# Edresson/VoiceSplit

Measured on AMD Instinct MI355X. Metric: utterances/sec (3 s clips, B=64/GPU) fwd+bwd, channels-last bf16 activations / tape, bf16 MFMA, fp32 accumulate / statistics / master weights, higher is better.
Workload: dtype bf16 (conv activations and tape stored as bf16; bf16 MFMA operands in the convs, the LSTM / head contractions and the BPTT, f16 operands in the forward recurrence; fp32 accumulate, BatchNorm statistics, gate arithmetic / cell state, loss head, master weights)

## Files before the change

### voicesplit_amd/csrc/audio.hip

```cpp
#include <math.h>

#include "../../include/voicesplit_hip.h"
#include "stft_common.h"

namespace {

__global__ __launch_bounds__(256)
void reim_to_features_kernel(const float* __restrict__ reim, float* __restrict__ spec, float* __restrict__ phase, VsStftShape s) {
  const long long n = (long long)s.B * s.T * s.F;
  for (long long i = (long long)blockIdx.x * 256 + threadIdx.x; i < n; i += (long long)gridDim.x * 256) {
    const long long m = i / s.F;
    const int f = (int)(i - m * s.F);
    const float re = reim[m * s.ldk + f], im = reim[m * s.ldk + s.F + f];
    const float mag = sqrtf(re * re + im * im);
    const float db = 20.0f * log10f(fmaxf(1e-5f, mag)) - s.ref_level_db;
    spec[i] = fminf(fmaxf(db / (-s.min_level_db), -1.0f), 0.0f) + 1.0f;
    if (phase) phase[i] = atan2f(im, re);
  }
}

}

extern "C" {

size_t vs_audio_workspace_bytes(const vs_loss_dims* d) { return vs_sisnr_workspace_bytes(d); }

int vs_wav_to_spec(const vs_loss_dims* d, const float* wav, float* spec, float* phase, void* ws, size_t ws_bytes, void* stream_) {
  hipStream_t stream = (hipStream_t)stream_;
  VsStftShape s;
  if (int rc = vs_stft_make_shape(d, &s)) return rc;
  s.periodic = 1;
  const VsStftLayout L = vs_stft_layout(s);
  VS_REQUIRE(wav && spec, "wav_to_spec: NULL argument");
  VS_REQUIRE(s.S > s.n_fft / 2, "wav_to_spec: clip shorter than the reflect padding");
  VS_REQUIRE(ws && (reinterpret_cast<uintptr_t>(ws) & 255) == 0 && ws_bytes >= L.total, "wav_to_spec: workspace too small or misaligned (%zu < %zu)", ws_bytes, L.total);
  const int M = s.B * s.T;
  float* frames = at<float>(ws, L.frames_e);
  float* basis = at<float>(ws, L.fbasis);
  float* reim = at<float>(ws, L.reim_e);
  const bool split = vs_stft_split(s);
  unsigned* amax = at<unsigned>(ws, L.amax);
  float* scales = at<float>(ws, L.scales);
  if (split) VS_CHECK_HIP(hipMemsetAsync(amax, 0, (size_t)VS_AMAX_SLOTS * 4, stream));
  vs_stft_frames_launch(wav, frames, s, split ? amax : nullptr, vs_grid_for((long long)M * s.win, split ? 2048 : 16384), stream);
  vs_stft_basis_launch(basis, s, scales + 6, stream);
  if (split) if (int rc = vs_scale_from_absmax_impl(amax, VS_AMAX_SLOTS, scales, stream)) return rc;
  if (int rc = vs_stft_contract(split, 0, frames, s.win, basis, s.win, reim, s.ldk, M, s.K, s.win, scales, scales + 6, stream)) return rc;
  hipLaunchKernelGGL(reim_to_features_kernel, dim3(vs_grid_for((long long)M * s.F, 16384)), dim3(256), 0, stream, reim, spec, phase, s);
  VS_LAUNCH_CHECK();
  return 0;
}

int vs_spec_to_wav(const vs_loss_dims* d, const float* spec, const float* mask, const float* phase, float* wav,
                   void* ws, size_t ws_bytes, void* stream_) {
  hipStream_t stream = (hipStream_t)stream_;
  VsStftShape s;
  if (int rc = vs_stft_make_shape(d, &s)) return rc;
  s.periodic = 1;
  s.true_phase = 1;
  const VsStftLayout L = vs_stft_layout(s);
  VS_REQUIRE(spec && phase && wav, "spec_to_wav: NULL argument");
  if (int rc = vs_stft_check_envelope(s)) return rc;
  VS_REQUIRE(ws && (reinterpret_cast<uintptr_t>(ws) & 255) == 0 && ws_bytes >= L.total, "spec_to_wav: workspace too small or misaligned (%zu < %zu)", ws_bytes, L.total);
  const int M = s.B * s.T;
  float* basis = at<float>(ws, L.basis);
  float* env = at<float>(ws, L.env);
  float* reim = at<float>(ws, L.reim_e);
  float* frames = at<float>(ws, L.frames_e);
  const bool split = vs_stft_split(s);
  unsigned* amax = at<unsigned>(ws, L.amax);
  float* scales = at<float>(ws, L.scales);
  vs_istft_basis_launch(basis, s, scales + 6, stream);
  vs_istft_envelope_launch(env, s, stream);
  if (split) VS_CHECK_HIP(hipMemsetAsync(amax, 0, (size_t)VS_AMAX_SLOTS * 4, stream));
  vs_spec_to_reim_launch(spec, mask, phase, reim, s, split ? amax : nullptr, vs_grid_for((long long)M * s.F, split ? 2048 : 16384), stream);
  if (split) if (int rc = vs_scale_from_absmax_impl(amax, VS_AMAX_SLOTS, scales, stream)) return rc;
  if (int rc = vs_stft_contract(split, 0, reim, s.ldk, basis, s.ldk, frames, s.win, M, s.win, s.K, scales, scales + 6, stream)) return rc;
  vs_overlap_add_launch(frames, env, wav, s, stream);
  VS_LAUNCH_CHECK();
  return 0;
}

}
```

### voicesplit_amd/csrc/conv_f16x3.hip

```cpp
#include "conv_f16x3_common.h"
#include "vs_internal.h"

namespace {

constexpr int kPadTaps = 2;

__global__ __launch_bounds__(256)
void absmax_kernel(const float* __restrict__ x, long long n, unsigned* __restrict__ out) {
  float m = 0.f;
  const long long n4 = n >> 2;
  const float4* x4 = reinterpret_cast<const float4*>(x);
  for (long long i = (long long)blockIdx.x * 256 + threadIdx.x; i < n4; i += (long long)gridDim.x * 256) {
    const float4 v = x4[i];
    m = fmaxf(m, fmaxf(fmaxf(fabsf(v.x), fabsf(v.y)), fmaxf(fabsf(v.z), fabsf(v.w))));
  }
  if (blockIdx.x == 0 && threadIdx.x < (n & 3)) m = fmaxf(m, fabsf(x[(n4 << 2) + threadIdx.x]));
#pragma unroll
  for (int o = 32; o > 0; o >>= 1) m = fmaxf(m, __shfl_down(m, o, 64));
  if ((threadIdx.x & 63) == 0) atomicMax(out, __float_as_uint(m));
}

__global__ void scale_from_absmax_kernel(const unsigned* __restrict__ amax, int n, float* __restrict__ scale) {
  unsigned mb = 0;
  for (int i = threadIdx.x; i < n; i += 64) mb = amax[i] > mb ? amax[i] : mb;
#pragma unroll
  for (int o = 32; o > 0; o >>= 1) { const unsigned other = __shfl_down(mb, o, 64); mb = other > mb ? other : mb; }
  if (threadIdx.x != 0) return;
  const float m = __uint_as_float(mb);
  int e = 0;
  float s = 1.f, inv = 1.f;
  if (m > 0.f && m < 3.0e38f) {
    (void)frexpf(m, &e);
    int k = 10 - e;
    k = k > 100 ? 100 : (k < -100 ? -100 : k);
    s = ldexpf(1.f, k);
    inv = ldexpf(1.f, -k);
  }
  scale[0] = s;
  scale[1] = inv;
}

__global__ void conv_pack_weights_f16_kernel(const float* __restrict__ w, _Float16* __restrict__ wp, int KT, int KF,
                                             int transpose_flip, const float* __restrict__ wscale) {
  const int NT = KT * KF;
  const int total = kNChunk * NT * 2 * 2 * 64 * 8;
  int idx = blockIdx.x * blockDim.x + threadIdx.x;
  if (idx >= total + kPadTaps * (kTapBytes / 2)) return;
  if (idx >= total) { wp[idx] = (_Float16)0.f; return; }
  const int j = idx & 7;
  const int lane = (idx >> 3) & 63;
  const int part = (idx >> 9) & 1;
  const int cb = (idx >> 10) & 1;
  const int tg = idx >> 11;
  const int chunk = tg / NT, tap = tg - chunk * NT;
  const int kt = tap / KF, kf = tap - kt * KF;
  const int co = cb * 32 + (lane & 31);
  const int ci = chunk * kChunk + 8 * (lane >> 5) + j;
  const float v = (transpose_flip ? w[((ci * kCi + co) * KT + (KT - 1 - kt)) * KF + (KF - 1 - kf)]
                                  : w[((co * kCi + ci) * KT + kt) * KF + kf]) * wscale[0];
  f16x2 hi, lo;
  split2(v, 0.f, hi, lo);
  wp[idx] = part ? lo[0] : hi[0];
}

template <int KT, int KF, int P, int ACT, bool STATS = false>
__global__ __launch_bounds__(256, 2)
void conv64_f16x3_kernel(const float* __restrict__ in, const _Float16* __restrict__ wp,
                         const float* __restrict__ scale, const float* __restrict__ shift,
                         const float* __restrict__ in_scale, const float* __restrict__ w_scale,
                         float* __restrict__ out, int T, int F, int dil, int n_rt, int n_ft, unsigned* amax_out,
                         int i_base, int i_end,
                         double* bn_stats = nullptr) {
  constexpr int R = 4 * P;
  constexpr int ROWS = R + KT - 1;
  constexpr int PX = kTileF + KF - 1 + ((kTileF + KF - 1) % 4 ? 4 - (kTileF + KF - 1) % 4 : 0);
  constexpr int NPIX = ROWS * PX;
  constexpr int NPP = (NPIX + 255) / 256;
  constexpr int NT = KT * KF;
  constexpr int GT = KF == 1 ? KT : KF;
  constexpr int NGRP = NT / GT;
  __shared__ __attribute__((aligned(16))) u32x4 sIn[(NPIX + (P + 1) * PX) * 4];
  constexpr int NWBUF = NGRP > 1 ? 2 : 1;
  __shared__ __attribute__((aligned(16))) u32x4 sW[NWBUF][GT * kTapVec];

  const int tid = threadIdx.x;
  const int lane = tid & 63;
  const int wave = __builtin_amdgcn_readfirstlane(tid >> 6);
  const int l31 = lane & 31;
  const int half = lane >> 5;

  int bid = blockIdx.x;
  const int ft = bid % n_ft; bid /= n_ft;
  const int rt = bid % n_rt; bid /= n_rt;
  const int cls = bid % dil;
  const int b = bid / dil;
  const int n_all = (T - cls + dil - 1) / dil;
  const int n_c = n_all < i_end ? n_all : i_end;
  const int i0 = i_base + rt * R;
  if (i0 >= n_c) return;
  const int f0 = ft * kTileF;
  const size_t plane = (size_t)T * F;
  const float* in_b = in + (size_t)b * kCi * plane;
  const unsigned plane_bytes = (unsigned)(plane * sizeof(float));
  const unsigned slab_bytes = plane_bytes * kChunk;
  const float s_in = in_scale[0];
  const float inv = in_scale[1] * w_scale[1];

  unsigned voff[NPP];
#pragma unroll
  for (int i = 0; i < NPP; ++i) {
    const int pix = tid + 256 * i;
    const int rr = pix / PX;
    const int x = pix - rr * PX;
    const int iin = i0 - KT / 2 + rr;
    const int f = f0 - KF / 2 + x;
    const bool ok = (pix < NPIX) && (iin >= 0) && (iin < n_all) && (f >= 0) && (f < F);
    voff[i] = ok ? (unsigned)(((cls + dil * iin) * F + f) * 4) : kOob;
  }
  float stage[NPP][kChunk];
  auto load_chunk = [&](int chunk) {
    const float* src = in_b + (size_t)chunk * kChunk * plane;
    __amdgpu_buffer_rsrc_t rsrc = __builtin_amdgcn_make_buffer_rsrc(const_cast<float*>(src), 0, slab_bytes, 0x00020000);
#pragma unroll
    for (int i = 0; i < NPP; ++i)
#pragma unroll
      for (int c = 0; c < kChunk; ++c)
        stage[i][c] = __builtin_bit_cast(float, __builtin_amdgcn_raw_buffer_load_b32(rsrc, voff[i], c * plane_bytes, 0));
  };
  auto store_chunk = [&]() {
#pragma unroll
    for (int i = 0; i < NPP; ++i) {
      const int pix = tid + 256 * i;
      if (pix < NPIX) {
        const int sw = ((pix % PX) >> 2) & 3;
#pragma unroll
        for (int h = 0; h < 2; ++h) {
          f16x2 hi[4], lo[4];
#pragma unroll
          for (int q = 0; q < 4; ++q) split2(stage[i][8 * h + 2 * q] * s_in, stage[i][8 * h + 2 * q + 1] * s_in, hi[q], lo[q]);
          u32x4 vh, vl;
#pragma unroll
          for (int q = 0; q < 4; ++q) {
            vh[q] = __builtin_bit_cast(unsigned, hi[q]);
            vl[q] = __builtin_bit_cast(unsigned, lo[q]);
          }
          sIn[pix * 4 + ((0 + h) ^ sw)] = vh;
          sIn[pix * 4 + ((2 + h) ^ sw)] = vl;
        }
      }
    }
  };

  __amdgpu_buffer_rsrc_t wrsrc = __builtin_amdgcn_make_buffer_rsrc(
      const_cast<_Float16*>(wp), 0, (unsigned)((kNChunk * NT + kPadTaps) * kTapBytes), 0x00020000);
  u32x4 wreg[GT];
  auto load_w = [&](int gg) {
#pragma unroll
    for (int i = 0; i < GT; ++i)
      wreg[i] = __builtin_amdgcn_raw_buffer_load_b128(wrsrc, (unsigned)((tid + 256 * i) * 16), gg * (GT * kTapBytes), 0);
  };
  auto store_w = [&](int buf) {
#pragma unroll
    for (int i = 0; i < GT; ++i) sW[buf][tid + 256 * i] = wreg[i];
  };

  f32x16 acc[2][P];
#pragma unroll
  for (int cb = 0; cb < 2; ++cb)
#pragma unroll
    for (int p = 0; p < P; ++p)
#pragma unroll
      for (int r = 0; r < 16; ++r) acc[cb][p][r] = 0.f;

  const bool wave_active = (i0 + wave * P) < n_c;
  auto load_a = [&](int buf, int g, u32x4 (&a)[2][2]) {
#pragma unroll
    for (int cb = 0; cb < 2; ++cb)
#pragma unroll
      for (int part = 0; part < 2; ++part) a[cb][part] = sW[buf][g * kTapVec + (cb * 2 + part) * 64 + lane];
  };
  const u32x4* bbase[KF][2];
#pragma unroll
  for (int kf = 0; kf < KF; ++kf) {
    const int x = l31 + kf;
    const int sw = (x >> 2) & 3;
    bbase[kf][0] = sIn + ((wave * P) * PX + x) * 4 + ((0 + half) ^ sw);
    bbase[kf][1] = sIn + ((wave * P) * PX + x) * 4 + ((2 + half) ^ sw);
  }
  auto load_b = [&](int kt, int kf, u32x4 (&bf)[P][2]) {
#pragma unroll
    for (int p = 0; p < P; ++p) {
      bf[p][0] = bbase[kf][0][(p + kt) * PX * 4];
      bf[p][1] = bbase[kf][1][(p + kt) * PX * 4];
    }
  };

  load_w(0);
  load_chunk(0);
  int gg = 0;
#pragma unroll 1
  for (int chunk = 0; chunk < kNChunk; ++chunk) {
    __syncthreads();
    store_chunk();
#pragma unroll
    for (int grp = 0; grp < NGRP; ++grp, ++gg) {
      const int buf = NWBUF > 1 ? (gg & 1) : 0;
      store_w(buf);
      __syncthreads();
      if (gg + 1 < kNChunk * NGRP) load_w(gg + 1);
      if (grp == 0 && chunk + 1 < kNChunk) load_chunk(chunk + 1);
      if (wave_active) {
        u32x4 a_cur[2][2], a_nxt[2][2], b_cur[P][2], b_nxt[P][2];
        const int kt0 = KF == 1 ? 0 : grp;
        load_a(buf, 0, a_cur);
        load_b(kt0, 0, b_cur);
#pragma unroll
        for (int g = 0; g < GT; ++g) {
          const int gn = g + 1 < GT ? g + 1 : g;
          load_a(buf, gn, a_nxt);
          load_b(KF == 1 ? gn : kt0, KF == 1 ? 0 : gn, b_nxt);
          __builtin_amdgcn_sched_barrier(0);
#pragma unroll
          for (int term = 0; term < 3; ++term) {
#pragma unroll
            for (int p = 0; p < P; ++p) {
              const f16x8 bq = __builtin_bit_cast(f16x8, b_cur[p][term == 1 ? 1 : 0]);
#pragma unroll
              for (int cb = 0; cb < 2; ++cb) {
                const f16x8 aq = __builtin_bit_cast(f16x8, a_cur[cb][term == 0 ? 1 : 0]);
                acc[cb][p] = __builtin_amdgcn_mfma_f32_32x32x16_f16(aq, bq, acc[cb][p], 0, 0, 0);
              }
            }
          }
          __builtin_amdgcn_sched_barrier(0);
#pragma unroll
          for (int cb = 0; cb < 2; ++cb)
#pragma unroll
            for (int part = 0; part < 2; ++part) a_cur[cb][part] = a_nxt[cb][part];
#pragma unroll
          for (int p = 0; p < P; ++p) { b_cur[p][0] = b_nxt[p][0]; b_cur[p][1] = b_nxt[p][1]; }
        }
      }
    }
  }

  if (!STATS && !wave_active) return;
  const int f = f0 + l31;
  float* out_b = out + (size_t)b * kCo * plane;
  float m = 0.f;
  float stS[2][16], stQ[2][16];
#pragma unroll
  for (int cb = 0; cb < 2; ++cb) {
#pragma unroll
    for (int r = 0; r < 16; ++r) {
      const int co = cb * 32 + (r & 3) + 8 * (r >> 2) + 4 * half;
      const float sc = scale[co] * inv, sh = shift[co];
      stS[cb][r] = 0.f; stQ[cb][r] = 0.f;
#pragma unroll
      for (int p = 0; p < P; ++p) {
        const int i = i0 + wave * P + p;
        if (wave_active && i < n_c && f < F) {
          const int t = cls + dil * i;
          const float y = vs_act_fast<ACT>(fmaf(acc[cb][p][r], sc, sh));
          out_b[(size_t)co * plane + (size_t)t * F + f] = y;
          m = fmaxf(m, fabsf(y));
          if (STATS) { stS[cb][r] += y; stQ[cb][r] = fmaf(y, y, stQ[cb][r]); }
        }
      }
    }
  }
  vs_absmax_commit(m, amax_out);
  if (STATS) {
#pragma unroll
    for (int cb = 0; cb < 2; ++cb)
#pragma unroll
      for (int r = 0; r < 16; ++r) {
        float sv = stS[cb][r], qv = stQ[cb][r];
#pragma unroll
        for (int o = 16; o > 0; o >>= 1) { sv += __shfl_xor(sv, o, 64); qv += __shfl_xor(qv, o, 64); }
        stS[cb][r] = sv; stQ[cb][r] = qv;
      }
    __syncthreads();
    float* red = reinterpret_cast<float*>(sIn);
    if (l31 == 0) {
#pragma unroll
      for (int cb = 0; cb < 2; ++cb)
#pragma unroll
        for (int r = 0; r < 16; ++r) {
          const int co = cb * 32 + (r & 3) + 8 * (r >> 2) + 4 * half;
          red[(wave * 64 + co) * 2 + 0] = stS[cb][r];
          red[(wave * 64 + co) * 2 + 1] = stQ[cb][r];
        }
    }
    __syncthreads();
    if (tid < 128) {
      const double v = (double)red[tid] + (double)red[128 + tid] + (double)red[256 + tid] + (double)red[384 + tid];
      atomicAdd(bn_stats + (size_t)(blockIdx.x % VS_BN_STAT_SLOTS) * 128 + tid, v);
    }
  }
}

template <int KT, int KF, int P>
int launch_conv(const float* in, const _Float16* wp, const float* scale, const float* shift, const float* in_scale,
                const float* w_scale, float* out, int B, int T, int F, int dil, int act, unsigned* amax_out, hipStream_t stream,
                int i_base = 0, int i_end = 0x7fffffff, double* bn_stats = nullptr) {
  constexpr int R = 4 * P;
  const int rows_all = (T + dil - 1) / dil;
  const int rows_max = (rows_all < i_end ? rows_all : i_end) - i_base;
  const int n_rt = (rows_max + R - 1) / R;
  const int n_ft = (F + kTileF - 1) / kTileF;
  const long long nblk = (long long)B * dil * n_rt * n_ft;
  VS_REQUIRE(nblk > 0 && nblk < 2147483647LL, "conv64_f16x3: grid of %lld blocks out of range", nblk);
  dim3 grid((unsigned)nblk), block(256);
  auto launch = [&](auto A, auto S) {
    hipLaunchKernelGGL((conv64_f16x3_kernel<KT, KF, P, decltype(A)::value, decltype(S)::value>), grid, block, 0, stream, in, wp, scale, shift,
                       in_scale, w_scale, out, T, F, dil, n_rt, n_ft, amax_out, i_base, i_end, bn_stats);
  };
  if (bn_stats) {
    VS_REQUIRE(act == VS_ACT_NONE, "conv64_f16x3: fused BatchNorm statistics need act = NONE");
    launch(std::integral_constant<int, VS_ACT_NONE>(), std::true_type());
  } else if (int rc = conv_f16x3_dispatch_act(act, "conv64_f16x3", [&](auto A) { launch(A, std::false_type()); })) {
    return rc;
  }
  VS_LAUNCH_CHECK();
  return 0;
}

long long tile_rows(int T, int dil, int R) {
  long long tot = 0;
  for (int c = 0; c < dil && c < T; ++c) {
    int n = (T - c + dil - 1) / dil;
    tot += (long long)((n + R - 1) / R) * R;
  }
  return tot;
}

}

extern "C" size_t vs_conv64_packed_f16_floats(int KT, int KF) { return (size_t)(kNChunk * KT * KF + kPadTaps) * (kTapBytes / 4); }

int vs_scale_from_absmax_impl(const unsigned* amax, int n, float* scale2, hipStream_t stream) {
  hipLaunchKernelGGL(scale_from_absmax_kernel, dim3(1), dim3(64), 0, stream, amax, n, scale2);
  VS_LAUNCH_CHECK();
  return 0;
}

int vs_absmax_accum_impl(const float* x, long long n, unsigned* amax, hipStream_t stream) {
  VS_REQUIRE(n > 0, "absmax: n=%lld", n);
  VS_REQUIRE((reinterpret_cast<uintptr_t>(x) & 15) == 0, "absmax: tensor must be 16-byte aligned");
  const long long nb = ((n >> 2) + 255) / 256;
  hipLaunchKernelGGL(absmax_kernel, dim3((unsigned)(nb < 2048 ? (nb > 0 ? nb : 1) : 2048)), dim3(256), 0, stream, x, n, amax);
  VS_LAUNCH_CHECK();
  return 0;
}

int vs_pow2_scale_impl(const float* x, long long n, unsigned* amax_scratch, float* scale2, hipStream_t stream) {
  VS_REQUIRE(n > 0, "pow2_scale: n=%lld", n);
  VS_REQUIRE((reinterpret_cast<uintptr_t>(x) & 15) == 0, "pow2_scale: tensor must be 16-byte aligned");
  VS_CHECK_HIP(hipMemsetAsync(amax_scratch, 0, sizeof(unsigned), stream));
  const long long nb = ((n >> 2) + 255) / 256;
  hipLaunchKernelGGL(absmax_kernel, dim3((unsigned)(nb < 2048 ? (nb > 0 ? nb : 1) : 2048)), dim3(256), 0, stream, x, n, amax_scratch);
  return vs_scale_from_absmax_impl(amax_scratch, 1, scale2, stream);
}

int vs_conv64_pack_f16_impl(const float* w, _Float16* wp, int KT, int KF, int transpose_flip, unsigned* amax_scratch,
                            float* w_scale2, hipStream_t stream) {
  VS_REQUIRE((KT == 7 && KF == 1) || (KT == 5 && KF == 5), "conv64_f16x3: unsupported kernel %dx%d", KT, KF);
  if (int rc = vs_pow2_scale_impl(w, (long long)kCo * kCi * KT * KF, amax_scratch, w_scale2, stream)) return rc;
  const int total = (int)(vs_conv64_packed_f16_floats(KT, KF) * 2);
  hipLaunchKernelGGL(conv_pack_weights_f16_kernel, dim3((total + 255) / 256), dim3(256), 0, stream, w, wp, KT, KF, transpose_flip, w_scale2);
  VS_LAUNCH_CHECK();
  return 0;
}

static int g_conv_kernel = 0;
extern "C" int vs_set_conv_kernel(int mode) {
  if (mode < 0 || mode > 2) return -1;
  g_conv_kernel = mode;
  return 0;
}

int vs_conv64_f16x3_fwd_impl(const float* in, const _Float16* wp, const float* scale, const float* shift,
                             const float* in_scale2, const float* w_scale2, float* out,
                             int B, int T, int F, int KT, int KF, int dil, int act, unsigned* amax_out, hipStream_t stream,
                             double* bn_stats) {
  VS_REQUIRE(B > 0 && T > 0 && F > 0 && dil > 0, "conv64_f16x3: bad shape B=%d T=%d F=%d dil=%d", B, T, F, dil);
  VS_REQUIRE((long long)kChunk * T * F * 4 < (long long)kOob, "conv64_f16x3: T*F=%lld too large for 32-bit slab offsets", (long long)T * F);
  VS_REQUIRE((KT == 7 && KF == 1) || (KT == 5 && KF == 5), "conv64_f16x3: unsupported kernel %dx%d", KT, KF);
  const bool p2 = tile_rows(T, dil, 8) * 100 <= tile_rows(T, dil, 4) * 112;
  const int all = 0x7fffffff;
#define VS_ONE_TILE(KT_, KF_, P_, I0_, I1_) \
  launch_conv<KT_, KF_, P_>(in, wp, scale, shift, in_scale2, w_scale2, out, B, T, F, dil, act, amax_out, stream, I0_, I1_, bn_stats)
  if (KT == 7) return p2 ? VS_ONE_TILE(7, 1, 2, 0, all) : VS_ONE_TILE(7, 1, 1, 0, all);
  const int rows_all = (T + dil - 1) / dil, full8 = rows_all / 8 * 8, rem = rows_all - full8;
  const bool tail = full8 > 0 && rem > 0 && rem <= 4;
  const int body_end = tail ? full8 : all;
  int rc;
  if (g_conv_kernel != 1 && (long long)kCo * T * F * 4 < (long long)kOob) {
    rc = vs_conv64_f16x3_pk_impl(in, wp, scale, shift, in_scale2, w_scale2, out, B, T, F, dil, act, amax_out, stream,
                                 g_conv_kernel == 2 ? vs_opt(VS_OPT_ABLATION) : 0, body_end, bn_stats);
  } else {
    rc = tail || p2 ? VS_ONE_TILE(5, 5, 2, 0, body_end) : VS_ONE_TILE(5, 5, 1, 0, body_end);
  }
  if (rc || !tail) return rc;
  return VS_ONE_TILE(5, 5, 1, full8, all);
#undef VS_ONE_TILE
}
```

### voicesplit_amd/csrc/gemm_f16x3.hip

```cpp
#include <stdlib.h>

#include "vs_internal.h"

namespace {

typedef _Float16 h8 __attribute__((ext_vector_type(8)));
typedef _Float16 h2 __attribute__((ext_vector_type(2)));
typedef unsigned u2v __attribute__((ext_vector_type(2)));
typedef unsigned u4v __attribute__((ext_vector_type(4)));

constexpr int BM = 128, BN = 128;
constexpr int pitch_of(int BK) { return BK / 2 + 2; }
constexpr int regs_of(int BK) { return BM * BK / 256; }

struct Gemm16Args {
  const float* A; int lda;
  const float* W; int ldw;
  const float* W_hi; int n_split;
  float* C; int ldc;
  int M, N, K;
  const float* bias1;
  const float* bias2;
  const float* rowbias;
  int ldrb, group;
  const float* gate; int ldg;
  int a_relu, w_relu, act, accumulate;
  const float* a_scale;
  const float* w_scale;
  int tiles_m, tiles_n;
  int band;
};

template <bool BF = false>
__device__ __forceinline__ void split_pair(float x0, float x1, unsigned& hi, unsigned& lo) {
  if (BF) { hi = vs_pack_bf16(x0, x1); lo = 0u; return; }
  const h2 h = __builtin_bit_cast(h2, __builtin_amdgcn_cvt_pkrtz(x0, x1));
  const h2 l = __builtin_bit_cast(h2, __builtin_amdgcn_cvt_pkrtz(x0 - (float)h[0], x1 - (float)h[1]));
  hi = __builtin_bit_cast(unsigned, h);
  lo = __builtin_bit_cast(unsigned, l);
}

template <bool BF, class HV>
__device__ __forceinline__ f32x16 g_mma(HV a, HV b, f32x16 c, int, int, int) {
  if (BF) return __builtin_amdgcn_mfma_f32_32x32x16_bf16(__builtin_bit_cast(vs_bf16x8, a), __builtin_bit_cast(vs_bf16x8, b), c, 0, 0, 0);
  return __builtin_amdgcn_mfma_f32_32x32x16_f16(a, b, c, 0, 0, 0);
}

struct OperandView {
  __amdgpu_buffer_rsrc_t lo, hi;
  int row_lo, rows_lo;
  int row_hi, rows_hi;
  int use_lo, use_hi;
};

constexpr unsigned kOob = 0xFFFFFFF0u;

__device__ __forceinline__ bool gemm_tile_of(int tiles_m, int tiles_n, int band_rows, int& tm, int& tn) {
  const int per = (int)(gridDim.x >> 3);
  const int t = (int)(blockIdx.x & 7) * per + (int)(blockIdx.x >> 3);
  if (t >= tiles_m * tiles_n) return false;
  if (band_rows <= 0) { tm = t / tiles_n; tn = t - tm * tiles_n; return true; }
  const int band_tiles = band_rows * tiles_n;
  const int band = t / band_tiles;
  const int r = t - band * band_tiles;
  const int rows = min(band_rows, tiles_m - band * band_rows);
  tn = r / rows;
  tm = band * band_rows + (r - tn * rows);
  return true;
}

template <int LAYOUT, bool VEC, int BK>
__device__ __forceinline__ void tile_load(float (&r)[regs_of(BK)], const OperandView& o, int ld, int row0_kmajor, int k0, int K, int tid) {
  constexpr int RT = regs_of(BK);
  typedef float f4 __attribute__((ext_vector_type(4)));
  if (LAYOUT == 0) {
#pragma unroll
    for (int i = 0; i < RT / 4; ++i) {
      const int v = tid + 256 * i;
      const int lr = v / (BK / 4), c4 = k0 + (v % (BK / 4)) * 4;
      f4 t = {0.f, 0.f, 0.f, 0.f};
      auto fetch = [&](const __amdgpu_buffer_rsrc_t rs, int row, int nrows) {
        const bool okr = row >= 0 && row < nrows;
        const unsigned base = ((unsigned)row * (unsigned)ld + (unsigned)c4) * 4u;
        if (VEC) {
          return __builtin_bit_cast(f4, __builtin_amdgcn_raw_buffer_load_b128(rs, (okr && c4 < K) ? base : kOob, 0, 0));
        } else {
          f4 q;
#pragma unroll
          for (int e = 0; e < 4; ++e)
            q[e] = __builtin_bit_cast(float, __builtin_amdgcn_raw_buffer_load_b32(rs, (okr && c4 + e < K) ? base + 4u * e : kOob, 0, 0));
          return q;
        }
      };
      if (o.use_lo) t = fetch(o.lo, o.row_lo + lr, o.rows_lo);
      if (o.use_hi) t += fetch(o.hi, o.row_hi + lr, o.rows_hi);
      r[4 * i + 0] = t[0]; r[4 * i + 1] = t[1]; r[4 * i + 2] = t[2]; r[4 * i + 3] = t[3];
    }
  } else {
    const unsigned voff = ((unsigned)(2 * (tid >> 7)) * (unsigned)ld + (unsigned)(tid & 127)) * 4u;
    const unsigned so0 = ((unsigned)k0 * (unsigned)ld + (unsigned)row0_kmajor) * 4u;
#pragma unroll
    for (int i = 0; i < RT / 2; ++i) {
      const unsigned so = so0 + (unsigned)(4 * i) * (unsigned)ld * 4u;
      r[2 * i + 0] = __builtin_bit_cast(float, __builtin_amdgcn_raw_buffer_load_b32(o.lo, voff, so, 0));
      r[2 * i + 1] = __builtin_bit_cast(float, __builtin_amdgcn_raw_buffer_load_b32(o.lo, voff, so + (unsigned)ld * 4u, 0));
    }
  }
}

template <int LAYOUT, int BK, bool BF = false>
__device__ __forceinline__ void tile_store(const float (&r)[regs_of(BK)], unsigned* __restrict__ sh, unsigned* __restrict__ sl,
                                           float s, bool relu, int tid) {
  constexpr int RT = regs_of(BK), PW = pitch_of(BK);
  const float floor_ = relu ? 0.f : -__builtin_inff();
  if (LAYOUT == 0) {
#pragma unroll
    for (int i = 0; i < RT / 4; ++i) {
      const int v = tid + 256 * i;
      float x[4];
#pragma unroll
      for (int j = 0; j < 4; ++j) x[j] = fmaxf(r[4 * i + j], floor_) * s;
      unsigned h0, l0, h1, l1;
      split_pair<BF>(x[0], x[1], h0, l0);
      split_pair<BF>(x[2], x[3], h1, l1);
      u2v hi, lo;
      hi[0] = h0; hi[1] = h1;
      lo[0] = l0; lo[1] = l1;
      *reinterpret_cast<u2v*>(&sh[(v / (BK / 4)) * PW + (v % (BK / 4)) * 2]) = hi;
      *reinterpret_cast<u2v*>(&sl[(v / (BK / 4)) * PW + (v % (BK / 4)) * 2]) = lo;
    }
  } else {
#pragma unroll
    for (int i = 0; i < RT / 2; ++i) {
      const int idx = tid + 256 * i;
      const float x0 = fmaxf(r[2 * i], floor_) * s;
      const float x1 = fmaxf(r[2 * i + 1], floor_) * s;
      unsigned hi, lo;
      split_pair<BF>(x0, x1, hi, lo);
      sh[(idx & 127) * PW + (idx >> 7)] = hi;
      sl[(idx & 127) * PW + (idx >> 7)] = lo;
    }
  }
}

template <int LA, int LB, bool VEC, int BK, int OCC, bool BF = false>
__global__ __launch_bounds__(256, OCC)
void gemm_f16x3_kernel(Gemm16Args g) {
  constexpr int RT = regs_of(BK), PW = pitch_of(BK);
  __shared__ __attribute__((aligned(16))) unsigned sAh[BM * PW], sAl[BM * PW], sWh[BN * PW], sWl[BN * PW];

  const int tid = threadIdx.x;
  const int lane = tid & 63;
  const int wave = tid >> 6;
  const int wm = wave >> 1, wn = wave & 1;
  const int l31 = lane & 31, half = lane >> 5;
  int tile_m, tile_n;
  if (!gemm_tile_of(g.tiles_m, g.tiles_n, g.band, tile_m, tile_n)) return;
  const int m0 = tile_m * BM, n0 = tile_n * BN;
  const float sa = g.a_scale[0], sw = g.w_scale[0];
  const float inv = g.a_scale[1] * g.w_scale[1];

  f32x16 acc[2][2];
#pragma unroll
  for (int a = 0; a < 2; ++a)
#pragma unroll
    for (int b = 0; b < 2; ++b)
#pragma unroll
      for (int r = 0; r < 16; ++r) acc[a][b][r] = 0.f;

  float ra[RT], rw[RT];
  auto desc = [](const float* p, size_t floats) {
    return __builtin_amdgcn_make_buffer_rsrc(const_cast<float*>(p), 0, (int)(floats * 4), 0x00020000);
  };
  OperandView va, vw;
  va.lo = va.hi = desc(g.A, LA ? (size_t)(g.K - 1) * g.lda + g.M : (size_t)(g.M - 1) * g.lda + g.K);
  va.row_lo = m0; va.rows_lo = g.M; va.row_hi = 0; va.rows_hi = 0; va.use_lo = 1; va.use_hi = 0;
  const int nlo = g.n_split < g.N ? g.n_split : g.N;
  vw.lo = desc(g.W, LB ? (size_t)(g.K - 1) * g.ldw + g.N : (size_t)(nlo - 1) * g.ldw + g.K);
  vw.hi = (!LB && g.N > nlo) ? desc(g.W_hi, (size_t)(g.N - nlo - 1) * g.ldw + g.K) : vw.lo;
  vw.row_lo = n0; vw.rows_lo = nlo; vw.row_hi = n0 - nlo; vw.rows_hi = g.N - nlo;
  vw.use_lo = LB || n0 < nlo; vw.use_hi = !LB && n0 + BN > nlo && g.N > nlo;

  const int fa = (wm * 64 + l31) * PW + 4 * half;
  const int fw = (wn * 64 + l31) * PW + 4 * half;

  tile_load<LA, VEC, BK>(ra, va, g.lda, m0, 0, g.K, tid);
  tile_load<LB, VEC, BK>(rw, vw, g.ldw, n0, 0, g.K, tid);
  for (int k0 = 0; k0 < g.K; k0 += BK) {
    __syncthreads();
    tile_store<LA, BK, BF>(ra, sAh, sAl, sa, g.a_relu != 0, tid);
    tile_store<LB, BK, BF>(rw, sWh, sWl, sw, g.w_relu != 0, tid);
    __syncthreads();
    if (k0 + BK < g.K) {
      tile_load<LA, VEC, BK>(ra, va, g.lda, m0, k0 + BK, g.K, tid);
      tile_load<LB, VEC, BK>(rw, vw, g.ldw, n0, k0 + BK, g.K, tid);
    }
#pragma unroll
    for (int ks = 0; ks < BK / 16; ++ks) {
      h8 ah[2], al[2], bh[2], bl[2];
#pragma unroll
      for (int x = 0; x < 2; ++x) {
        const int oa = fa + x * 32 * PW + 8 * ks, ow = fw + x * 32 * PW + 8 * ks;
        u4v t;
        u2v p0 = *reinterpret_cast<const u2v*>(&sAh[oa]), p1 = *reinterpret_cast<const u2v*>(&sAh[oa + 2]);
        t[0] = p0[0]; t[1] = p0[1]; t[2] = p1[0]; t[3] = p1[1];
        ah[x] = __builtin_bit_cast(h8, t);
        p0 = *reinterpret_cast<const u2v*>(&sAl[oa]); p1 = *reinterpret_cast<const u2v*>(&sAl[oa + 2]);
        t[0] = p0[0]; t[1] = p0[1]; t[2] = p1[0]; t[3] = p1[1];
        al[x] = __builtin_bit_cast(h8, t);
        p0 = *reinterpret_cast<const u2v*>(&sWh[ow]); p1 = *reinterpret_cast<const u2v*>(&sWh[ow + 2]);
        t[0] = p0[0]; t[1] = p0[1]; t[2] = p1[0]; t[3] = p1[1];
        bh[x] = __builtin_bit_cast(h8, t);
        p0 = *reinterpret_cast<const u2v*>(&sWl[ow]); p1 = *reinterpret_cast<const u2v*>(&sWl[ow + 2]);
        t[0] = p0[0]; t[1] = p0[1]; t[2] = p1[0]; t[3] = p1[1];
        bl[x] = __builtin_bit_cast(h8, t);
      }
#pragma unroll
      for (int term = BF ? 2 : 0; term < 3; ++term)
#pragma unroll
        for (int mb = 0; mb < 2; ++mb)
#pragma unroll
          for (int nb = 0; nb < 2; ++nb)
            acc[mb][nb] = g_mma<BF>(term == 0 ? al[mb] : ah[mb], term == 1 ? bl[nb] : bh[nb],
                                                                 acc[mb][nb], 0, 0, 0);
    }
  }

#pragma unroll
  for (int nb = 0; nb < 2; ++nb) {
    const int n = n0 + wn * 64 + nb * 32 + l31;
    if (n >= g.N) continue;
    float bcol = 0.f;
    if (g.bias1) bcol += g.bias1[n];
    if (g.bias2) bcol += g.bias2[n];
#pragma unroll
    for (int mb = 0; mb < 2; ++mb) {
#pragma unroll
      for (int r = 0; r < 16; ++r) {
        const int m = m0 + wm * 64 + mb * 32 + (r & 3) + 8 * (r >> 2) + 4 * half;
        if (m < g.M) {
          float v = fmaf(acc[mb][nb][r], inv, bcol);
          if (g.rowbias) v += g.rowbias[(size_t)(m / g.group) * g.ldrb + n];
          v = vs_act_rt(v, g.act);
          if (g.gate) v = g.gate[(size_t)m * g.ldg + n] > 0.f ? v : 0.f;
          float* c = g.C + (size_t)m * g.ldc + n;
          if (g.accumulate) v += *c;
          *c = v;
        }
      }
    }
  }
}

template <int LA, int LB>
void launch_layout(const Gemm16Args& g, bool vec, dim3 grid, hipStream_t stream, bool bf) {
  if (bf) {
    if (vec) hipLaunchKernelGGL((gemm_f16x3_kernel<LA, LB, true, 32, 3, true>), grid, dim3(256), 0, stream, g);
    else hipLaunchKernelGGL((gemm_f16x3_kernel<LA, LB, false, 32, 3, true>), grid, dim3(256), 0, stream, g);
    return;
  }
  if (vec) hipLaunchKernelGGL((gemm_f16x3_kernel<LA, LB, true, 32, 3>), grid, dim3(256), 0, stream, g);
  else hipLaunchKernelGGL((gemm_f16x3_kernel<LA, LB, false, 32, 3>), grid, dim3(256), 0, stream, g);
}

constexpr int PBK = VS_GEMM_KPAD;
constexpr int PPW = PBK / 2 + 4;
constexpr int PCPR = PBK / 8;
constexpr int PRPP = 256 / PCPR;
constexpr int PNP = 128 / PRPP;

__global__ __launch_bounds__(256)
void split_rows_kernel(const float* __restrict__ src, int rows, int K, int ld, const float* __restrict__ scale,
                       _Float16* __restrict__ hi, _Float16* __restrict__ lo, int Kp, int relu, int bf) {
  const float s = scale[0];
  const int groups = Kp >> 3;
  const long long total = (long long)rows * groups;
  for (long long i = (long long)blockIdx.x * 256 + threadIdx.x; i < total; i += (long long)gridDim.x * 256) {
    const long long r = i / groups;
    const int k0 = (int)(i - r * groups) * 8;
    const float* p = src + r * ld + k0;
    float x[8];
#pragma unroll
    for (int e = 0; e < 8; ++e) {
      float v = (k0 + e < K) ? p[e] : 0.f;
      if (relu) v = fmaxf(v, 0.f);
      x[e] = v * s;
    }
    u4v h, l;
#pragma unroll
    for (int q = 0; q < 4; ++q) {
      unsigned hq, lq;
      if (bf) split_pair<true>(x[2 * q], x[2 * q + 1], hq, lq);
      else split_pair<false>(x[2 * q], x[2 * q + 1], hq, lq);
      h[q] = hq;
      l[q] = lq;
    }
    *reinterpret_cast<u4v*>(hi + r * Kp + k0) = h;
    *reinterpret_cast<u4v*>(lo + r * Kp + k0) = l;
  }
}

struct GemmPreArgs {
  const _Float16* Ah; const _Float16* Al;
  const _Float16* Wh; const _Float16* Wl;
  float* C; int ldc;
  int M, N, Kp;
  const float* bias1; const float* bias2;
  const float* rowbias; int ldrb, group;
  int act, accumulate;
  const float* a_scale; const float* w_scale;
  int tiles_m, tiles_n;
  int band;
};

template <bool BF>
__global__ __launch_bounds__(256, 2)
void gemm_pre_kernel(GemmPreArgs g) {
  __shared__ __attribute__((aligned(16))) unsigned sAh[BM * PPW], sAl[BM * PPW], sWh[BN * PPW], sWl[BN * PPW];
  const int tid = threadIdx.x;
  const int lane = tid & 63;
  const int wave = tid >> 6;
  const int wm = wave >> 1, wn = wave & 1;
  const int l31 = lane & 31, half = lane >> 5;
  int tile_m, tile_n;
  if (!gemm_tile_of(g.tiles_m, g.tiles_n, g.band, tile_m, tile_n)) return;
  const int m0 = tile_m * BM, n0 = tile_n * BN;
  const float inv = g.a_scale[1] * g.w_scale[1];

  f32x16 acc[2][2];
#pragma unroll
  for (int a = 0; a < 2; ++a)
#pragma unroll
    for (int b = 0; b < 2; ++b)
#pragma unroll
      for (int r = 0; r < 16; ++r) acc[a][b][r] = 0.f;

  auto desc = [](const _Float16* p, size_t halves) {
    return __builtin_amdgcn_make_buffer_rsrc(const_cast<_Float16*>(p), 0, (int)(halves * 2), 0x00020000);
  };
  const __amdgpu_buffer_rsrc_t rAh = desc(g.Ah, (size_t)g.M * g.Kp), rAl = desc(g.Al, (size_t)g.M * g.Kp);
  const __amdgpu_buffer_rsrc_t rWh = desc(g.Wh, (size_t)g.N * g.Kp), rWl = desc(g.Wl, (size_t)g.N * g.Kp);
  const int srow = tid / PCPR, sq = tid % PCPR;
  unsigned offA[PNP], offW[PNP];
#pragma unroll
  for (int i = 0; i < PNP; ++i) {
    const int row = srow + PRPP * i;
    offA[i] = (m0 + row < g.M) ? (unsigned)(((size_t)(m0 + row) * g.Kp + 8 * sq) * 2) : kOob;
    offW[i] = (n0 + row < g.N) ? (unsigned)(((size_t)(n0 + row) * g.Kp + 8 * sq) * 2) : kOob;
  }
  u4v ra[PNP][2], rw[PNP][2];
  auto tile_load = [&](int k0) {
    const unsigned so = (unsigned)k0 * 2u;
#pragma unroll
    for (int i = 0; i < PNP; ++i) {
      ra[i][0] = __builtin_amdgcn_raw_buffer_load_b128(rAh, offA[i], so, 0);
      ra[i][1] = __builtin_amdgcn_raw_buffer_load_b128(rAl, offA[i], so, 0);
      rw[i][0] = __builtin_amdgcn_raw_buffer_load_b128(rWh, offW[i], so, 0);
      rw[i][1] = __builtin_amdgcn_raw_buffer_load_b128(rWl, offW[i], so, 0);
    }
  };
  const int st = srow * PPW + 4 * sq;
  auto tile_store = [&]() {
#pragma unroll
    for (int i = 0; i < PNP; ++i) {
      *reinterpret_cast<u4v*>(&sAh[st + PRPP * i * PPW]) = ra[i][0];
      *reinterpret_cast<u4v*>(&sAl[st + PRPP * i * PPW]) = ra[i][1];
      *reinterpret_cast<u4v*>(&sWh[st + PRPP * i * PPW]) = rw[i][0];
      *reinterpret_cast<u4v*>(&sWl[st + PRPP * i * PPW]) = rw[i][1];
    }
  };
  const int fa = (wm * 64 + l31) * PPW + 4 * half;
  const int fw = (wn * 64 + l31) * PPW + 4 * half;

  tile_load(0);
  for (int k0 = 0; k0 < g.Kp; k0 += PBK) {
    __syncthreads();
    tile_store();
    __syncthreads();
    if (k0 + PBK < g.Kp) tile_load(k0 + PBK);
#pragma unroll
    for (int ks = 0; ks < PBK / 16; ++ks) {
      h8 ah[2], al[2], bh[2], bl[2];
#pragma unroll
      for (int x = 0; x < 2; ++x) {
        const int oa = fa + x * 32 * PPW + 8 * ks, ow = fw + x * 32 * PPW + 8 * ks;
        ah[x] = __builtin_bit_cast(h8, *reinterpret_cast<const u4v*>(&sAh[oa]));
        al[x] = __builtin_bit_cast(h8, *reinterpret_cast<const u4v*>(&sAl[oa]));
        bh[x] = __builtin_bit_cast(h8, *reinterpret_cast<const u4v*>(&sWh[ow]));
        bl[x] = __builtin_bit_cast(h8, *reinterpret_cast<const u4v*>(&sWl[ow]));
      }
#pragma unroll
      for (int term = BF ? 2 : 0; term < 3; ++term)
#pragma unroll
        for (int mb = 0; mb < 2; ++mb)
#pragma unroll
          for (int nb = 0; nb < 2; ++nb)
            acc[mb][nb] = g_mma<BF>(term == 0 ? al[mb] : ah[mb], term == 1 ? bl[nb] : bh[nb],
                                                                 acc[mb][nb], 0, 0, 0);
    }
  }

#pragma unroll
  for (int nb = 0; nb < 2; ++nb) {
    const int n = n0 + wn * 64 + nb * 32 + l31;
    if (n >= g.N) continue;
    float bcol = 0.f;
    if (g.bias1) bcol += g.bias1[n];
    if (g.bias2) bcol += g.bias2[n];
#pragma unroll
    for (int mb = 0; mb < 2; ++mb) {
#pragma unroll
      for (int r = 0; r < 16; ++r) {
        const int m = m0 + wm * 64 + mb * 32 + (r & 3) + 8 * (r >> 2) + 4 * half;
        if (m < g.M) {
          float v = fmaf(acc[mb][nb][r], inv, bcol);
          if (g.rowbias) v += g.rowbias[(size_t)(m / g.group) * g.ldrb + n];
          v = vs_act_rt(v, g.act);
          float* c = g.C + (size_t)m * g.ldc + n;
          if (g.accumulate) v += *c;
          *c = v;
        }
      }
    }
  }
}

bool aligned16(const void* p) { return (reinterpret_cast<uintptr_t>(p) & 15) == 0; }

int gemm_band() { return 8; }

}

int vs_pow2_scale_impl(const float* x, long long n, unsigned* amax_scratch, float* scale2, hipStream_t stream);

int vs_gemm_f16x3_impl(int layout_a, int layout_w, const float* A, int lda, const float* W, const float* W_hi,
                       int n_split, int ldw, float* C, int ldc, int M, int N, int K,
                       const float* bias1, const float* bias2, const float* rowbias, int ldrb, int group,
                       const float* gate, int ldg, int a_relu, int w_relu, int act, int accumulate,
                       const float* a_scale2, const float* w_scale2, hipStream_t stream, int math) {
  const bool bf = math == VS_MATH_CODE_BF16;
  VS_REQUIRE(M > 0 && N > 0 && K > 0, "gemm_f16x3: bad shape M=%d N=%d K=%d", M, N, K);
  VS_REQUIRE((layout_a == 0 || layout_a == 1) && (layout_w == 0 || layout_w == 1), "gemm_f16x3: bad layout");
  VS_REQUIRE(lda >= (layout_a ? M : K) && ldw >= (layout_w ? N : K) && ldc >= N,
             "gemm_f16x3: leading dims lda=%d ldw=%d ldc=%d vs M=%d N=%d K=%d", lda, ldw, ldc, M, N, K);
  VS_REQUIRE(!rowbias || (group > 0 && ldrb >= N), "gemm_f16x3: rowbias needs group>0 and ldrb>=N");
  VS_REQUIRE(!gate || ldg >= N, "gemm_f16x3: gate needs ldg>=N");
  VS_REQUIRE(act == VS_ACT_NONE || act == VS_ACT_RELU || act == VS_ACT_SIGMOID, "gemm_f16x3: unsupported activation %d", act);
  VS_REQUIRE(layout_w == 0 || (W_hi == nullptr || n_split >= N), "gemm_f16x3: stacked W needs the K-contiguous layout");
  VS_REQUIRE(n_split >= N || W_hi != nullptr, "gemm_f16x3: W_hi is NULL but n_split=%d < N=%d", n_split, N);
  VS_REQUIRE(a_scale2 && w_scale2, "gemm_f16x3: NULL scale");
  VS_REQUIRE(!layout_a || ((size_t)(K - 1) * lda + M) * 4 < (1ull << 32), "gemm_f16x3: K-major A above 4 GiB");
  VS_REQUIRE(!layout_w || ((size_t)(K - 1) * ldw + N) * 4 < (1ull << 32), "gemm_f16x3: K-major W above 4 GiB");
  Gemm16Args g{A, lda, W, ldw, W_hi, n_split, C, ldc, M, N, K, bias1, bias2, rowbias, ldrb, group > 0 ? group : 1,
               gate, ldg, a_relu, w_relu, act, accumulate, a_scale2, w_scale2, (M + BM - 1) / BM, (N + BN - 1) / BN, gemm_band()};
  const bool vec = (lda % 4 == 0) && (ldw % 4 == 0) && (K % 4 == 0) && aligned16(A) && aligned16(W) && aligned16(W_hi);
  VS_REQUIRE(layout_a || ((size_t)(M - 1) * lda + K) * 4 < (1ull << 32) - 64, "gemm_f16x3: A above 4 GiB");
  VS_REQUIRE(layout_w || ((size_t)(N - 1) * ldw + K) * 4 < (1ull << 32) - 64, "gemm_f16x3: W above 4 GiB");
  VS_REQUIRE((long long)g.tiles_m * g.tiles_n < (1LL << 30), "gemm_f16x3: too many tiles");
  dim3 grid((unsigned)((g.tiles_m * g.tiles_n + 7) / 8 * 8));
  if (layout_a == 0 && layout_w == 0) launch_layout<0, 0>(g, vec, grid, stream, bf);
  else if (layout_a == 0 && layout_w == 1) launch_layout<0, 1>(g, vec, grid, stream, bf);
  else if (layout_a == 1 && layout_w == 0) launch_layout<1, 0>(g, vec, grid, stream, bf);
  else launch_layout<1, 1>(g, vec, grid, stream, bf);
  VS_LAUNCH_CHECK();
  return 0;
}

size_t vs_gemm_presplit_bytes(int M, int N, int K) {
  const size_t Kp = (size_t)(K + PBK - 1) / PBK * PBK;
  return ((size_t)M + (size_t)N) * Kp * 2 * sizeof(_Float16) + 1024;
}

int vs_split_rows_impl(const float* x, int rows, int K, int ld, const float* scale2, _Float16* hi, _Float16* lo, int relu,
                       hipStream_t stream, int math) {
  VS_REQUIRE(rows > 0 && K > 0 && ld >= K, "split_rows: bad shape rows=%d K=%d ld=%d", rows, K, ld);
  const int Kp = (K + PBK - 1) / PBK * PBK;
  const long long total = (long long)rows * (Kp >> 3);
  const long long nb = (total + 255) / 256;
  hipLaunchKernelGGL(split_rows_kernel, dim3((unsigned)(nb < 4096 ? nb : 4096)), dim3(256), 0, stream, x, rows, K, ld, scale2, hi, lo, Kp, relu,
                     math == VS_MATH_CODE_BF16 ? 1 : 0);
  VS_LAUNCH_CHECK();
  return 0;
}

int vs_gemm_presplit_impl(const _Float16* Ah, const _Float16* Al, const _Float16* Wh, const _Float16* Wl, int Kp,
                          float* C, int ldc, int M, int N, const float* bias1, const float* bias2,
                          const float* rowbias, int ldrb, int group, int act, int accumulate,
                          const float* a_scale2, const float* w_scale2, hipStream_t stream, int math) {
  VS_REQUIRE(M > 0 && N > 0 && Kp > 0 && Kp % PBK == 0 && ldc >= N, "gemm_presplit: bad shape M=%d N=%d Kp=%d ldc=%d", M, N, Kp, ldc);
  VS_REQUIRE(((size_t)M * Kp) * 2 < (1ull << 32) - 64 && ((size_t)N * Kp) * 2 < (1ull << 32) - 64, "gemm_presplit: operand above 4 GiB");
  VS_REQUIRE(!rowbias || (group > 0 && ldrb >= N), "gemm_presplit: rowbias needs group>0 and ldrb>=N");
  VS_REQUIRE(aligned16(Ah) && aligned16(Al) && aligned16(Wh) && aligned16(Wl), "gemm_presplit: operands must be 16-byte aligned");
  GemmPreArgs g{Ah, Al, Wh, Wl, C, ldc, M, N, Kp, bias1, bias2, rowbias, ldrb, group > 0 ? group : 1, act, accumulate,
                a_scale2, w_scale2, (M + BM - 1) / BM, (N + BN - 1) / BN, gemm_band()};
  if (math == VS_MATH_CODE_BF16) hipLaunchKernelGGL(gemm_pre_kernel<true>, dim3((unsigned)((g.tiles_m * g.tiles_n + 7) / 8 * 8)), dim3(256), 0, stream, g);
  else hipLaunchKernelGGL(gemm_pre_kernel<false>, dim3((unsigned)((g.tiles_m * g.tiles_n + 7) / 8 * 8)), dim3(256), 0, stream, g);
  VS_LAUNCH_CHECK();
  return 0;
}
```

### voicesplit_amd/csrc/griffin_lim.hip

```cpp
#include <math.h>

#include "../../include/voicesplit_hip.h"
#include "stft_common.h"

namespace {

__device__ __forceinline__ double gl_block_sum(double v) {
  __shared__ double red[4];
#pragma unroll
  for (int o = 32; o > 0; o >>= 1) v += __shfl_down(v, o, 64);
  if ((threadIdx.x & 63) == 0) red[threadIdx.x >> 6] = v;
  __syncthreads();
  return (red[0] + red[1]) + (red[2] + red[3]);
}

__global__ __launch_bounds__(256)
void gl_item_max_kernel(const float* __restrict__ a, const float* __restrict__ b, unsigned* __restrict__ vmax, VsStftShape s) {
  const int item = blockIdx.y;
  const int n = s.T * s.F;
  const size_t base = (size_t)item * n;
  float m = 0.f;
  for (int i = blockIdx.x * 256 + threadIdx.x; i < n; i += gridDim.x * 256) {
    float v = a[base + i];
    if (b) v *= b[base + i];
    m = fmaxf(m, fminf(fmaxf(v, 0.f), 1.f));
  }
#pragma unroll
  for (int o = 32; o > 0; o >>= 1) m = fmaxf(m, __shfl_down(m, o, 64));
  if ((threadIdx.x & 63) == 0) atomicMax(&vmax[item], __float_as_uint(m));
}

__global__ __launch_bounds__(256)
void gl_target_kernel(const float* __restrict__ a, const float* __restrict__ b, const float* __restrict__ phase, float power,
                      float* __restrict__ S, float* __restrict__ reim, double* __restrict__ den, VsStftShape s,
                      unsigned* __restrict__ amax, const unsigned* __restrict__ vmax, float* __restrict__ gain) {
  const int item = blockIdx.y;
  const int n = s.T * s.F;
  const size_t base = (size_t)item * n;
  const double kpow = 0.11512925464970228 * (double)power;
  int e = 0;
  (void)frexp(exp((((double)__uint_as_float(vmax[item]) - 1.0) * (-(double)s.min_level_db) + (double)s.ref_level_db) * kpow), &e);
  e = e > 120 ? 120 : (e < -120 ? -120 : e);
  const double level = ldexp(1.0, -e);
  if (blockIdx.x == 0 && threadIdx.x == 0) gain[item] = ldexpf(1.f, e);
  float mx = 0.f;
  double acc = 0.0;
  for (int i = blockIdx.x * 256 + threadIdx.x; i < n; i += gridDim.x * 256) {
    const int t = i / s.F, f = i - t * s.F;
    const size_t row = ((size_t)item * s.T + t) * s.ldk;
    double v = a[base + i];
    if (b) v *= (double)b[base + i];
    const double db = (fmin(fmax(v, 0.0), 1.0) - 1.0) * (-(double)s.min_level_db) + (double)s.ref_level_db;
    const float mag = (float)(exp(db * kpow) * level);
    float sn, cs;
    sincosf(phase[base + i], &sn, &cs);
    S[base + i] = mag;
    reim[row + f] = mag * cs;
    reim[row + s.F + f] = mag * sn;
    if (f == 0) for (int c = s.K; c < s.ldk; ++c) reim[row + c] = 0.f;
    mx = fmaxf(mx, mag);
    acc += (double)mag * (double)mag;
  }
  vs_absmax_commit(mx, amax);
  acc = gl_block_sum(acc);
  if (threadIdx.x == 0) atomicAdd(&den[item], acc);
}

__global__ __launch_bounds__(256)
void gl_project_kernel(float* __restrict__ reim, const float* __restrict__ S, double* __restrict__ num, unsigned* __restrict__ amax_reset,
                       VsStftShape s) {
  const int item = blockIdx.y;
  const int n = s.T * s.F;
  const size_t base = (size_t)item * n;
  if (amax_reset && blockIdx.x == 0 && item == 0)
    for (int i = threadIdx.x; i < VS_AMAX_SLOTS; i += 256) amax_reset[i] = 0u;
  double acc = 0.0;
  for (int i = blockIdx.x * 256 + threadIdx.x; i < n; i += gridDim.x * 256) {
    const int t = i / s.F, f = i - t * s.F;
    const size_t row = ((size_t)item * s.T + t) * s.ldk;
    const float re = reim[row + f], im = reim[row + s.F + f];
    const float tgt = S[base + i];
    const float n2 = re * re + im * im;
    float ore = tgt, oim = 0.f, mag = 0.f;
    if (n2 >= 1.17549435e-38f) {
      const float r = rsqrtf(n2);
      ore = tgt * (re * r);
      oim = tgt * (im * r);
      mag = n2 * r;
    }
    reim[row + f] = ore;
    reim[row + s.F + f] = oim;
    if (f == 0) for (int c = s.K; c < s.ldk; ++c) reim[row + c] = 0.f;
    const double d = (double)mag - (double)tgt;
    acc += d * d;
  }
  if (num) {
    acc = gl_block_sum(acc);
    if (threadIdx.x == 0) atomicAdd(&num[item], acc);
  }
}

__global__ __launch_bounds__(256)
void gl_reframe_kernel(const float* __restrict__ in, const float* __restrict__ env, float* __restrict__ out, VsStftShape s,
                       unsigned* __restrict__ amax) {
  const long long n = (long long)s.B * s.T * s.win;
  float mx = 0.f;
  for (long long i = (long long)blockIdx.x * 256 + threadIdx.x; i < n; i += (long long)gridDim.x * 256) {
    const long long m = i / s.win;
    const int j = (int)(i - m * s.win);
    const int b = (int)(m / s.T), t = (int)(m - (long long)b * s.T);
    int sp = s.hop * t - s.lead + j;
    if (sp < 0) sp = -sp;
    if (sp >= s.S) sp = 2 * (s.S - 1) - sp;
    const float v = hann_w(j, s) * (stft_gather(in, b, sp, s) / env[sp]);
    out[i] = v;
    mx = fmaxf(mx, fabsf(v));
  }
  vs_absmax_commit(mx, amax);
}

__global__ __launch_bounds__(256)
void gl_overlap_add_gain_kernel(const float* __restrict__ frames, const float* __restrict__ env, const float* __restrict__ gain,
                                float* __restrict__ wav, VsStftShape s) {
  const int sp = blockIdx.x * 256 + threadIdx.x;
  const int b = blockIdx.y;
  if (sp >= s.S) return;
  wav[(size_t)b * s.S + sp] = (stft_gather(frames, b, sp, s) / env[sp]) * gain[b];
}

__global__ void gl_residual_kernel(double* __restrict__ res, const double* __restrict__ den, int n_iter, int B) {
  const int i = blockIdx.x * blockDim.x + threadIdx.x;
  if (i >= n_iter * B) return;
  const double d = den[i % B];
  res[i] = d > 0.0 ? sqrt(res[i] / d) : 0.0;
}

int g_gl_reframe = 0;

}

extern "C" {

size_t vs_griffin_lim_workspace_bytes(const vs_loss_dims* d) { return vs_sisnr_workspace_bytes(d); }

int vs_set_griffin_lim_reframe(int mode) {
  VS_REQUIRE(mode >= 0 && mode <= 2, "vs_set_griffin_lim_reframe: mode %d (0 = default, 1 = overlap-add + framing, 2 = one gather launch)", mode);
  g_gl_reframe = mode;
  return 0;
}

int vs_griffin_lim(const vs_loss_dims* d, const float* spec, const float* mask, const float* init_phase, float power, int n_iter,
                   float* wav, double* residual, void* ws, size_t ws_bytes, void* stream_) {
  hipStream_t stream = (hipStream_t)stream_;
  VsStftShape s;
  if (int rc = vs_stft_make_shape(d, &s)) return rc;
  s.periodic = 1;
  s.true_phase = 1;
  const VsStftLayout L = vs_stft_layout(s);
  VS_REQUIRE(spec && init_phase && wav, "griffin_lim: NULL argument");
  VS_REQUIRE(n_iter >= 0, "griffin_lim: n_iter=%d", n_iter);
  VS_REQUIRE(power > 0.f && power < 3.0e38f, "griffin_lim: power=%g must be greater than 0", (double)power);
  VS_REQUIRE(s.S > s.n_fft / 2, "griffin_lim: clip shorter than the reflect padding");
  VS_REQUIRE((long long)s.T * s.F < (1ll << 31), "griffin_lim: T*F too large");
  if (int rc = vs_stft_check_envelope(s)) return rc;
  VS_REQUIRE(ws && (reinterpret_cast<uintptr_t>(ws) & 255) == 0 && ws_bytes >= L.total, "griffin_lim: workspace too small or misaligned (%zu < %zu)", ws_bytes, L.total);
  const int M = s.B * s.T;
  float* basis = at<float>(ws, L.basis);
  float* fbasis = at<float>(ws, L.fbasis);
  float* env = at<float>(ws, L.env);
  float* reim = at<float>(ws, L.reim_e);
  float* S = at<float>(ws, L.reim_t);
  float* frames = at<float>(ws, L.frames_e);
  float* frames2 = at<float>(ws, L.frames_t);
  double* den = at<double>(ws, L.mom);
  unsigned* vmax = at<unsigned>(ws, L.coef);
  float* gain = at<float>(ws, L.coef) + s.B;
  const bool split = vs_stft_split(s);
  unsigned* amax = at<unsigned>(ws, L.amax);
  float* scales = at<float>(ws, L.scales);
  const bool gather = g_gl_reframe != 1;
  vs_istft_basis_launch(basis, s, scales + 4, stream);
  vs_stft_basis_launch(fbasis, s, scales + 6, stream);
  vs_istft_envelope_launch(env, s, stream);
  if (split) VS_CHECK_HIP(hipMemsetAsync(amax, 0, (size_t)2 * VS_AMAX_SLOTS * 4, stream));
  VS_CHECK_HIP(hipMemsetAsync(den, 0, (size_t)s.B * 8, stream));
  VS_CHECK_HIP(hipMemsetAsync(vmax, 0, (size_t)s.B * 4, stream));
  const bool want_res = residual != nullptr && n_iter > 0;
  if (want_res) VS_CHECK_HIP(hipMemsetAsync(residual, 0, (size_t)n_iter * s.B * 8, stream));
  const int per_item = (s.T * s.F + 255) / 256;
  int gx = 2048 / s.B < 1 ? 1 : 2048 / s.B;
  if (gx > per_item) gx = per_item;
  const unsigned gfr = vs_grid_for((long long)M * s.win, split ? 2048 : 16384);
  auto istft = [&](float* out) {
    return vs_stft_contract(split, 0, reim, s.ldk, basis, s.ldk, out, s.win, M, s.win, s.K, scales + 2, scales + 4, stream);
  };
  hipLaunchKernelGGL(gl_item_max_kernel, dim3(gx, s.B), dim3(256), 0, stream, spec, mask, vmax, s);
  hipLaunchKernelGGL(gl_target_kernel, dim3(gx, s.B), dim3(256), 0, stream, spec, mask, init_phase, power, S, reim, den, s,
                     split ? amax + VS_AMAX_SLOTS : nullptr, vmax, gain);
  if (split) if (int rc = vs_scale_from_absmax_impl(amax + VS_AMAX_SLOTS, VS_AMAX_SLOTS, scales + 2, stream)) return rc;
  if (int rc = istft(frames)) return rc;
  for (int it = 0; it < n_iter; ++it) {
    float* cur = frames;
    if (gather) {
      hipLaunchKernelGGL(gl_reframe_kernel, dim3(gfr), dim3(256), 0, stream, frames, env, frames2, s, split ? amax : nullptr);
      cur = frames2;
    } else {
      vs_overlap_add_launch(frames, env, wav, s, stream);
      vs_stft_frames_launch(wav, frames, s, split ? amax : nullptr, gfr, stream);
    }
    if (split) if (int rc = vs_scale_from_absmax_impl(amax, VS_AMAX_SLOTS, scales, stream)) return rc;
    if (int rc = vs_stft_contract(split, 0, cur, s.win, fbasis, s.win, reim, s.ldk, M, s.K, s.win, scales, scales + 6, stream)) return rc;
    hipLaunchKernelGGL(gl_project_kernel, dim3(gx, s.B), dim3(256), 0, stream, reim, S, want_res ? residual + (size_t)it * s.B : nullptr,
                       split ? amax : nullptr, s);
    if (int rc = istft(frames)) return rc;
  }
  hipLaunchKernelGGL(gl_overlap_add_gain_kernel, dim3((s.S + 255) / 256, s.B), dim3(256), 0, stream, frames, env, gain, wav, s);
  if (want_res) hipLaunchKernelGGL(gl_residual_kernel, dim3((n_iter * s.B + 255) / 256), dim3(256), 0, stream, residual, den, n_iter, s.B);
  VS_LAUNCH_CHECK();
  return 0;
}

}
```

### voicesplit_amd/csrc/loss.hip

```cpp
#include <math.h>

#include "../../include/voicesplit_hip.h"
#include "stft_common.h"

namespace {

__global__ __launch_bounds__(256)
void overlap_add_bwd_kernel(const float* __restrict__ dwav, const float* __restrict__ env, float* __restrict__ dframes, VsStftShape s,
                            unsigned* __restrict__ amax = nullptr) {
  const long long n = (long long)s.B * s.T * s.win;
  float mx = 0.f;
  for (long long i = (long long)blockIdx.x * 256 + threadIdx.x; i < n; i += (long long)gridDim.x * 256) {
    const long long m = i / s.win;
    const int j = (int)(i - m * s.win);
    const int b = (int)(m / s.T), t = (int)(m - (long long)b * s.T);
    const int sp = s.hop * t - s.lead + j;
    const float v = (sp >= 0 && sp < s.S) ? dwav[(size_t)b * s.S + sp] / env[sp] : 0.f;
    dframes[i] = v;
    mx = fmaxf(mx, fabsf(v));
  }
  vs_absmax_commit(mx, amax);
}

__global__ __launch_bounds__(256)
void sisnr_moments_kernel(const float* __restrict__ est, const float* __restrict__ src, const int* __restrict__ len,
                          double* __restrict__ mom , VsStftShape s) {
  const int b = blockIdx.y;
  const int L = len ? (len[b] < s.S ? (len[b] > 0 ? len[b] : 0) : s.S) : s.S;
  double a[6] = {0, 0, 0, 0, 0, 0};
  for (int i = blockIdx.x * 256 + threadIdx.x; i < s.S; i += gridDim.x * 256) {
    const double e = est[(size_t)b * s.S + i], r = src[(size_t)b * s.S + i];
    a[0] += r;
    if (i < L) { a[1] += e; a[2] += r; a[3] += e * r; a[4] += e * e; a[5] += r * r; }
  }
  __shared__ double red[4][6];
#pragma unroll
  for (int q = 0; q < 6; ++q) {
#pragma unroll
    for (int o = 32; o > 0; o >>= 1) a[q] += __shfl_down(a[q], o, 64);
  }
  if ((threadIdx.x & 63) == 0) {
#pragma unroll
    for (int q = 0; q < 6; ++q) red[threadIdx.x >> 6][q] = a[q];
  }
  __syncthreads();
  if (threadIdx.x < 6) atomicAdd(&mom[b * 8 + threadIdx.x], (red[0][threadIdx.x] + red[1][threadIdx.x]) + (red[2][threadIdx.x] + red[3][threadIdx.x]));
}

__global__ void sisnr_finalize_kernel(const double* __restrict__ mom, const int* __restrict__ len, float* __restrict__ coef ,
                                      float* __restrict__ loss, VsStftShape s) {
  __shared__ double acc[64];
  const int tid = threadIdx.x;
  double part = 0.0;
  const double eps = 1e-16;
  for (int b = tid; b < s.B; b += 64) {
    const double nlen = len ? (double)len[b] : (double)s.S;
    const int Lm_i = len ? (len[b] < s.S ? (len[b] > 0 ? len[b] : 0) : s.S) : s.S;
    const double Lm = Lm_i;
    const double* m = mom + b * 8;
    const double mu_s = m[0] / nlen, mu_e = m[1] / nlen;
    const double Sze = m[1] - Lm * mu_e, Szs = m[2] - Lm * mu_s;
    const double dot = m[3] - mu_s * m[1] - mu_e * m[2] + Lm * mu_e * mu_s;
    const double Z = m[5] - 2 * mu_s * m[2] + Lm * mu_s * mu_s;
    const double E = m[4] - 2 * mu_e * m[1] + Lm * mu_e * mu_e;
    const double es = Z + eps;
    const double P = dot * dot * Z / (es * es);
    const double c = (es + eps) / (es * es);
    const double N = E - c * dot * dot + eps;
    const double snr = P / N;
    part += 10.0 * log10(snr + eps);
    const double k = 10.0 / (log(10.0) * (snr + eps)) * (-1.0 / s.B);
    const double gs = k * (2 * dot * Z / (es * es) / N + P / (N * N) * 2 * c * dot);
    const double ge = k * (-P / (N * N) * 2);
    const double gsum = gs * Szs + ge * Sze;
    float* o = coef + b * 8;
    o[0] = (float)gs; o[1] = (float)ge; o[2] = (float)(gsum / nlen); o[3] = (float)mu_s; o[4] = (float)mu_e;
    o[5] = (float)Lm_i;
  }
  acc[tid] = part;
  __syncthreads();
  if (tid == 0) {
    double t = 0;
    for (int i = 0; i < 64; ++i) t += acc[i];
    *loss = (float)(20.0 - t / s.B);
  }
}

__global__ __launch_bounds__(256)
void sisnr_grad_kernel(const float* __restrict__ est, const float* __restrict__ src, const float* __restrict__ coef,
                       float* __restrict__ dwav, VsStftShape s) {
  const int b = blockIdx.y;
  const float gs = coef[b * 8], ge = coef[b * 8 + 1], g0 = coef[b * 8 + 2], mu_s = coef[b * 8 + 3], mu_e = coef[b * 8 + 4];
  const int L = (int)coef[b * 8 + 5];
  for (int i = blockIdx.x * 256 + threadIdx.x; i < s.S; i += gridDim.x * 256) {
    float g = 0.f;
    if (i < L) {
      const float zs = src[(size_t)b * s.S + i] - mu_s, ze = est[(size_t)b * s.S + i] - mu_e;
      g = fmaf(gs, zs, fmaf(ge, ze, -g0));
    }
    dwav[(size_t)b * s.S + i] = g;
  }
}

__global__ __launch_bounds__(256)
void reim_to_dmask_kernel(const float* __restrict__ mixed, const float* __restrict__ mask, const float* __restrict__ phase,
                          const float* __restrict__ dreim, float* __restrict__ dmask, VsStftShape s) {
  const long long n = (long long)s.B * s.T * s.F;
  for (long long i = (long long)blockIdx.x * 256 + threadIdx.x; i < n; i += (long long)gridDim.x * 256) {
    const long long m = i / s.F;
    const int f = (int)(i - m * s.F);
    const float x = mixed[i], v = x * mask[i];
    float g = 0.f;
    if (v >= 0.f && v <= 1.f) {
      const float db = (v - 1.f) * (-s.min_level_db) + s.ref_level_db;
      const float mag = expf(db * kLn10Over20);
      float sn, cs;
      sincosf(phase[i], &sn, &cs);
      const float d = dreim[m * s.ldk + f] * expf(cs) + dreim[m * s.ldk + s.F + f] * expf(sn);
      g = x * (-s.min_level_db) * kLn10Over20 * mag * d;
    }
    dmask[i] = g;
  }
}

__global__ __launch_bounds__(256)
void powerlaw_kernel(const float* __restrict__ mixed, const float* __restrict__ mask, const float* __restrict__ target,
                     long long n, float power, float ratio, double* __restrict__ sums, float* __restrict__ dmask) {
  constexpr float kEps = 1e-16f;
  const float inv_n = (float)(1.0 / (double)n);
  double a0 = 0.0, a1 = 0.0;
  for (long long i = (long long)blockIdx.x * 256 + threadIdx.x; i < n; i += (long long)gridDim.x * 256) {
    const float mx = mixed[i];
    const float o = mx * mask[i] + kEps;
    const float t = target[i] + kEps;
    const float po = powf(o, power), pt = powf(t, power);
    const float ds = fabsf(pt) - fabsf(po), dc = pt - po;
    a0 += (double)(ds * ds);
    a1 += (double)(dc * dc);
    if (dmask) {
      const float sgn = po > 0.f ? 1.f : (po < 0.f ? -1.f : 0.f);
      const float dpo = (-2.f * ds * sgn - 2.f * ratio * dc) * inv_n;
      dmask[i] = mx * (power * powf(o, power - 1.f)) * dpo;
    }
  }
#pragma unroll
  for (int off = 32; off > 0; off >>= 1) {
    a0 += __shfl_down(a0, off, 64);
    a1 += __shfl_down(a1, off, 64);
  }
  __shared__ double sh[8];
  const int lane = threadIdx.x & 63, w = threadIdx.x >> 6;
  if (lane == 0) { sh[2 * w] = a0; sh[2 * w + 1] = a1; }
  __syncthreads();
  if (threadIdx.x == 0) {
    atomicAdd(&sums[0], sh[0] + sh[2] + sh[4] + sh[6]);
    atomicAdd(&sums[1], sh[1] + sh[3] + sh[5] + sh[7]);
  }
}

__global__ void powerlaw_finalize_kernel(const double* __restrict__ sums, long long n, float ratio, float* __restrict__ loss) {
  *loss = (float)(sums[0] / (double)n + (double)ratio * (sums[1] / (double)n));
}

}

extern "C" {

size_t vs_sisnr_workspace_bytes(const vs_loss_dims* d) {
  VsStftShape s;
  return vs_stft_make_shape(d, &s) ? 0 : vs_stft_layout(s).total;
}

int vs_sisnr_loss(const vs_loss_dims* d, const float* mixed, const float* mask, const float* target, const float* phase,
                  const int* seq_len, void* ws, size_t ws_bytes, float* loss, float* dmask, float* est_wav, void* stream_) {
  hipStream_t stream = (hipStream_t)stream_;
  VsStftShape s;
  if (int rc = vs_stft_make_shape(d, &s)) return rc;
  const VsStftLayout L = vs_stft_layout(s);
  VS_REQUIRE(mixed && mask && target && phase && loss, "sisnr_loss: NULL argument");
  if (int rc = vs_stft_check_envelope(s)) return rc;
  VS_REQUIRE(ws && (reinterpret_cast<uintptr_t>(ws) & 255) == 0 && ws_bytes >= L.total, "sisnr_loss: workspace too small or misaligned (%zu < %zu)", ws_bytes, L.total);
  const int M = s.B * s.T;
  const long long nspec = (long long)M * s.F;
  float* basis = at<float>(ws, L.basis);
  float* env = at<float>(ws, L.env);
  const bool split = vs_stft_split(s);
  unsigned* amax = at<unsigned>(ws, L.amax);
  float* scales = at<float>(ws, L.scales);
  vs_istft_basis_launch(basis, s, scales + 6, stream);
  vs_istft_envelope_launch(env, s, stream);
  float* reim[2] = {at<float>(ws, L.reim_e), at<float>(ws, L.reim_t)};
  float* frames[2] = {at<float>(ws, L.frames_e), at<float>(ws, L.frames_t)};
  float* wav[2] = {at<float>(ws, L.wav_e), at<float>(ws, L.wav_t)};
  if (split) VS_CHECK_HIP(hipMemsetAsync(amax, 0, (size_t)3 * VS_AMAX_SLOTS * 4, stream));
  const unsigned cap = split ? 2048 : 16384;
  vs_spec_to_reim_launch(mixed, mask, phase, reim[0], s, split ? amax : nullptr, vs_grid_for(nspec, cap), stream);
  vs_spec_to_reim_launch(target, nullptr, phase, reim[1], s, split ? amax + VS_AMAX_SLOTS : nullptr, vs_grid_for(nspec, cap), stream);
  for (int q = 0; q < 2; ++q) {
    if (split) if (int rc = vs_scale_from_absmax_impl(amax + q * VS_AMAX_SLOTS, VS_AMAX_SLOTS, scales + 2 * q, stream)) return rc;
    if (int rc = vs_stft_contract(split, 0, reim[q], s.ldk, basis, s.ldk, frames[q], s.win, M, s.win, s.K, scales + 2 * q, scales + 6, stream)) return rc;
    vs_overlap_add_launch(frames[q], env, wav[q], s, stream);
  }
  if (est_wav) VS_CHECK_HIP(hipMemcpyAsync(est_wav, wav[0], (size_t)s.B * s.S * 4, hipMemcpyDeviceToDevice, stream));
  double* mom = at<double>(ws, L.mom);
  float* coef = at<float>(ws, L.coef);
  VS_CHECK_HIP(hipMemsetAsync(mom, 0, (size_t)s.B * 8 * 8, stream));
  const int gx = vs_opt(VS_OPT_DETERMINISTIC) ? 1 : (s.S + 256 * 16 - 1) / (256 * 16);
  hipLaunchKernelGGL(sisnr_moments_kernel, dim3(gx, s.B), dim3(256), 0, stream, wav[0], wav[1], seq_len, mom, s);
  hipLaunchKernelGGL(sisnr_finalize_kernel, dim3(1), dim3(64), 0, stream, mom, seq_len, coef, loss, s);
  if (dmask) {
    float* dwav = at<float>(ws, L.dwav);
    hipLaunchKernelGGL(sisnr_grad_kernel, dim3(gx, s.B), dim3(256), 0, stream, wav[0], wav[1], coef, dwav, s);
    float* dframes = frames[0];
    hipLaunchKernelGGL(overlap_add_bwd_kernel, dim3(vs_grid_for((long long)M * s.win, cap)), dim3(256), 0, stream, dwav, env, dframes, s,
                       split ? amax + 2 * VS_AMAX_SLOTS : nullptr);
    float* dreim = reim[0];
    if (split) if (int rc = vs_scale_from_absmax_impl(amax + 2 * VS_AMAX_SLOTS, VS_AMAX_SLOTS, scales + 4, stream)) return rc;
    if (int rc = vs_stft_contract(split, 1, dframes, s.win, basis, s.ldk, dreim, s.ldk, M, s.K, s.win, scales + 4, scales + 6, stream)) return rc;
    hipLaunchKernelGGL(reim_to_dmask_kernel, dim3(vs_grid_for(nspec, 16384)), dim3(256), 0, stream, mixed, mask, phase, dreim, dmask, s);
  }
  VS_LAUNCH_CHECK();
  return 0;
}

int vs_powerlaw_loss(const float* mixed, const float* mask, const float* target, long long n, float power,
                     float complex_loss_ratio, double* scratch, float* loss, float* dmask, void* stream_) {
  hipStream_t stream = (hipStream_t)stream_;
  VS_REQUIRE(mixed && mask && target && scratch && loss, "powerlaw_loss: NULL argument");
  VS_REQUIRE(n > 0, "powerlaw_loss: n=%lld", n);
  VS_CHECK_HIP(hipMemsetAsync(scratch, 0, 2 * sizeof(double), stream));
  hipLaunchKernelGGL(powerlaw_kernel, dim3(vs_grid_for(n)), dim3(256), 0, stream, mixed, mask, target, n, power, complex_loss_ratio, scratch, dmask);
  hipLaunchKernelGGL(powerlaw_finalize_kernel, dim3(1), dim3(1), 0, stream, scratch, n, complex_loss_ratio, loss);
  VS_LAUNCH_CHECK();
  return 0;
}

}
```

### voicesplit_amd/csrc/stft.hip

```cpp
#include <math.h>

#include "../../include/voicesplit_hip.h"
#include "stft_common.h"

namespace {

__global__ void istft_basis_kernel(float* __restrict__ basis, VsStftShape s, float* __restrict__ scale2 = nullptr) {
  const int idx = blockIdx.x * blockDim.x + threadIdx.x;
  if (idx == 0 && scale2) {
    int e = 0;
    (void)frexpf(2.0f / (float)s.n_fft, &e);
    scale2[0] = ldexpf(1.f, 10 - e);
    scale2[1] = ldexpf(1.f, e - 10);
  }
  if (idx >= s.win * s.ldk) return;
  const int j = idx / s.ldk, k = idx - j * s.ldk;
  float v = 0.f;
  if (k < s.K) {
    const int kk = k < s.F ? k : k - s.F;
    const int n = (s.n_fft - s.win) / 2 + j;
    const int r = (int)(((long long)kk * n) % s.n_fft);
    float sn, cs;
    sincospif(2.0f * (float)r / (float)s.n_fft, &sn, &cs);
    const float c = (kk == 0 || 2 * kk == s.n_fft) ? 1.0f : 2.0f;
    v = (k < s.F ? cs : -sn) * c / (float)s.n_fft * hann_w(j, s);
  }
  basis[idx] = v;
}

__global__ void istft_envelope_kernel(float* __restrict__ env, VsStftShape s) {
  const int sp = blockIdx.x * blockDim.x + threadIdx.x;
  if (sp >= s.S) return;
  const int off = s.lead;
  float e = 0.f;
  int t_hi = (sp + off) / s.hop;
  if (t_hi > s.T - 1) t_hi = s.T - 1;
  for (int t = t_hi; t >= 0; --t) {
    const int j = sp - s.hop * t + off;
    if (j >= s.win) break;
    const float w = hann_w(j, s);
    e = fmaf(w, w, e);
  }
  env[sp] = e;
}

__global__ __launch_bounds__(256)
void spec_to_reim_kernel(const float* __restrict__ a, const float* __restrict__ b, const float* __restrict__ phase,
                         float* __restrict__ reim, VsStftShape s, unsigned* __restrict__ amax = nullptr) {
  const long long n = (long long)s.B * s.T * s.F;
  float mx = 0.f;
  for (long long i = (long long)blockIdx.x * 256 + threadIdx.x; i < n; i += (long long)gridDim.x * 256) {
    const long long m = i / s.F;
    const int f = (int)(i - m * s.F);
    float v = a[i];
    if (b) v *= b[i];
    const float db = (fminf(fmaxf(v, 0.f), 1.f) - 1.f) * (-s.min_level_db) + s.ref_level_db;
    const float mag = expf(db * kLn10Over20);
    float sn, cs;
    sincosf(phase[i], &sn, &cs);
    const float re = s.true_phase ? mag * cs : mag * expf(cs), im = s.true_phase ? mag * sn : mag * expf(sn);
    reim[m * s.ldk + f] = re;
    reim[m * s.ldk + s.F + f] = im;
    if (f == 0) for (int c = s.K; c < s.ldk; ++c) reim[m * s.ldk + c] = 0.f;
    mx = fmaxf(mx, fmaxf(fabsf(re), fabsf(im)));
  }
  vs_absmax_commit(mx, amax);
}

__global__ __launch_bounds__(256)
void stft_frames_kernel(const float* __restrict__ wav, float* __restrict__ frames, VsStftShape s, unsigned* __restrict__ amax = nullptr) {
  const long long n = (long long)s.B * s.T * s.win;
  float mx = 0.f;
  for (long long i = (long long)blockIdx.x * 256 + threadIdx.x; i < n; i += (long long)gridDim.x * 256) {
    const long long m = i / s.win;
    const int j = (int)(i - m * s.win);
    const int b = (int)(m / s.T), t = (int)(m - (long long)b * s.T);
    int idx = s.hop * t - s.lead + j;
    if (idx < 0) idx = -idx;
    if (idx >= s.S) idx = 2 * (s.S - 1) - idx;
    const float v = hann_w(j, s) * wav[(size_t)b * s.S + idx];
    frames[i] = v;
    mx = fmaxf(mx, fabsf(v));
  }
  vs_absmax_commit(mx, amax);
}

__global__ void stft_basis_kernel(float* __restrict__ basis, VsStftShape s, float* __restrict__ scale2 = nullptr) {
  const int idx = blockIdx.x * blockDim.x + threadIdx.x;
  if (idx == 0 && scale2) { scale2[0] = 512.f; scale2[1] = 1.f / 512.f; }
  if (idx >= s.K * s.win) return;
  const int k = idx / s.win, j = idx - k * s.win;
  const int kk = k < s.F ? k : k - s.F;
  const int n = (s.n_fft - s.win) / 2 + j;
  const int r = (int)(((long long)kk * n) % s.n_fft);
  float sn, cs;
  sincospif(2.0f * (float)r / (float)s.n_fft, &sn, &cs);
  basis[idx] = k < s.F ? cs : -sn;
}

__global__ __launch_bounds__(256)
void overlap_add_kernel(const float* __restrict__ frames, const float* __restrict__ env, float* __restrict__ wav, VsStftShape s) {
  const int sp = blockIdx.x * 256 + threadIdx.x;
  const int b = blockIdx.y;
  if (sp >= s.S) return;
  wav[(size_t)b * s.S + sp] = stft_gather(frames, b, sp, s) / env[sp];
}

}

void vs_istft_basis_launch(float* basis, const VsStftShape& s, float* scale2, hipStream_t stream) {
  hipLaunchKernelGGL(istft_basis_kernel, dim3((s.win * s.ldk + 255) / 256), dim3(256), 0, stream, basis, s, scale2);
}
void vs_istft_envelope_launch(float* env, const VsStftShape& s, hipStream_t stream) {
  hipLaunchKernelGGL(istft_envelope_kernel, dim3((s.S + 255) / 256), dim3(256), 0, stream, env, s);
}
void vs_stft_basis_launch(float* basis, const VsStftShape& s, float* scale2, hipStream_t stream) {
  hipLaunchKernelGGL(stft_basis_kernel, dim3((s.K * s.win + 255) / 256), dim3(256), 0, stream, basis, s, scale2);
}
void vs_stft_frames_launch(const float* wav, float* frames, const VsStftShape& s, unsigned* amax, unsigned grid, hipStream_t stream) {
  hipLaunchKernelGGL(stft_frames_kernel, dim3(grid), dim3(256), 0, stream, wav, frames, s, amax);
}
void vs_spec_to_reim_launch(const float* a, const float* b, const float* phase, float* reim, const VsStftShape& s, unsigned* amax, unsigned grid,
                            hipStream_t stream) {
  hipLaunchKernelGGL(spec_to_reim_kernel, dim3(grid), dim3(256), 0, stream, a, b, phase, reim, s, amax);
}
void vs_overlap_add_launch(const float* frames, const float* env, float* wav, const VsStftShape& s, hipStream_t stream) {
  hipLaunchKernelGGL(overlap_add_kernel, dim3((s.S + 255) / 256, s.B), dim3(256), 0, stream, frames, env, wav, s);
}

void vs_stft_fill_shape(const vs_loss_dims* d, int B, int T, int S, VsStftShape* s) {
  s->B = B; s->T = T; s->F = d->F; s->n_fft = d->n_fft; s->hop = d->hop; s->win = d->win;
  s->S = S;
  s->lead = d->n_fft / 2 - (d->n_fft - d->win) / 2;
  s->K = 2 * d->F;
  s->ldk = (s->K + 3) & ~3;
  s->min_level_db = d->min_level_db; s->ref_level_db = d->ref_level_db;
  s->periodic = 0; s->true_phase = 0;
}

int vs_stft_make_shape(const vs_loss_dims* d, VsStftShape* s) {
  VS_REQUIRE(d != nullptr, "loss dims is NULL");
  VS_REQUIRE(d->B > 0 && d->T > 1 && d->F > 1 && d->hop > 0 && d->win > 0, "loss: bad dims B=%d T=%d F=%d hop=%d win=%d", d->B, d->T, d->F, d->hop, d->win);
  VS_REQUIRE(d->n_fft == 2 * (d->F - 1), "loss: num_freq F=%d must be n_fft/2+1 (n_fft=%d)", d->F, d->n_fft);
  VS_REQUIRE(d->win <= d->n_fft && d->hop <= d->win, "loss: need hop <= win <= n_fft");
  VS_REQUIRE(d->B <= 65535, "loss: B too large");
  vs_stft_fill_shape(d, d->B, d->T, d->hop * (d->T - 1), s);
  return 0;
}

VsStftLayout vs_stft_layout(const VsStftShape& s) {
  VsStftLayout L;
  size_t off = 0;
  auto take = [&](size_t bytes) { size_t o = off; off = align_up(off + bytes); return o; };
  const size_t M = (size_t)s.B * s.T;
  L.basis = take((size_t)s.win * s.ldk * 4);
  L.fbasis = take((size_t)s.K * s.win * 4);
  L.env = take((size_t)s.S * 4);
  L.reim_e = take(M * s.ldk * 4);
  L.reim_t = take(M * s.ldk * 4);
  L.frames_e = take(M * s.win * 4);
  L.frames_t = take(M * s.win * 4);
  L.wav_e = take((size_t)s.B * s.S * 4);
  L.wav_t = take((size_t)s.B * s.S * 4);
  L.dwav = take((size_t)s.B * s.S * 4);
  L.mom = take((size_t)s.B * 8 * 8);
  L.coef = take((size_t)s.B * 8 * 4);
  L.amax = take((size_t)3 * VS_AMAX_SLOTS * 4);
  L.scales = take(4 * 2 * 4);
  L.total = off;
  return L;
}

int vs_stft_check_envelope(const VsStftShape& s) {
  static thread_local int c_key[5] = {0, 0, 0, 0, 0};
  static thread_local double c_min = 0.0;
  const int key[5] = {s.hop, s.win, s.T, s.periodic, 1};
  bool hit = true;
  for (int i = 0; i < 5; ++i) hit = hit && key[i] == c_key[i];
  if (!hit) {
    const int off = s.lead, den = s.periodic ? s.win : s.win - 1;
    auto env_at = [&](int sp) {
      double e = 0.0;
      int t_hi = (sp + off) / s.hop;
      if (t_hi > s.T - 1) t_hi = s.T - 1;
      for (int t = t_hi; t >= 0; --t) {
        const int j = sp - s.hop * t + off;
        if (j >= s.win) break;
        const double w = den > 0 ? 0.5 - 0.5 * cos(2.0 * 3.14159265358979323846 * (double)j / (double)den) : 1.0;
        e += w * w;
      }
      return e;
    };
    double mn = 1e300;
    const int span = s.win + s.hop;
    for (int sp = 0; sp < s.S; ++sp) {
      if (sp >= span && sp < s.S - span) { sp = s.S - span - 1; continue; }
      const double e = env_at(sp);
      if (e < mn) mn = e;
    }
    c_min = mn;
    for (int i = 0; i < 5; ++i) c_key[i] = key[i];
  }
  VS_REQUIRE(c_min > 1e-11, "istft: window envelope reaches %.3g (hop=%d win=%d %s Hann): the overlap-add would divide by zero; "
             "use hop <= win/2", c_min, s.hop, s.win, s.periodic ? "periodic" : "symmetric");
  return 0;
}

int vs_stft_contract(bool split, int layout_w, const float* A, int lda, const float* W, int ldw, float* C, int ldc, int M, int N, int K,
                     const float* a_scale2, const float* w_scale2, hipStream_t stream) {
  if (split)
    return vs_gemm_f16x3_impl(0, layout_w, A, lda, W, nullptr, 0x7fffffff, ldw, C, ldc, M, N, lda,
                              nullptr, nullptr, nullptr, 0, 1, nullptr, 0, 0, 0, VS_ACT_NONE, 0, a_scale2, w_scale2, stream,
                              VS_MATH_CODE_F16X3);
  return vs_gemm_general_impl(0, layout_w, A, lda, W, nullptr, 0x7fffffff, ldw, C, ldc, M, N, K,
                              nullptr, nullptr, nullptr, 0, 1, nullptr, 0, 0, 0, VS_ACT_NONE, 0, 0, 0, 1, nullptr, stream);
}
```

### voicesplit_amd/csrc/stft_common.h

```cpp
#pragma once
#include "vs_internal.h"

constexpr float kLn10Over20 = 0.11512925464970229f;

struct VsStftShape {
  int B, T, F, n_fft, hop, win, S;
  int lead;
  int K, ldk;
  float min_level_db, ref_level_db;
  int periodic;
  int true_phase;
};

struct VsStftLayout { size_t basis, fbasis, env, reim_e, reim_t, frames_e, frames_t, wav_e, wav_t, dwav, mom, coef, amax, scales, total; };

__device__ __forceinline__ float hann_w(int j, const VsStftShape& s) {
  const int den = s.periodic ? s.win : s.win - 1;
  return den > 0 ? 0.5f - 0.5f * cospif(2.0f * (float)j / (float)den) : 1.0f;
}

__device__ __forceinline__ float stft_gather(const float* __restrict__ frames, int b, int sp, const VsStftShape& s) {
  int t_hi = (sp + s.lead) / s.hop;
  if (t_hi > s.T - 1) t_hi = s.T - 1;
  float acc = 0.f;
  for (int t = t_hi; t >= 0; --t) {
    const int j = sp - s.hop * t + s.lead;
    if (j >= s.win) break;
    acc += frames[((size_t)b * s.T + t) * s.win + j];
  }
  return acc;
}

inline unsigned vs_grid_for(long long n, unsigned cap = 2048) {
  const long long nb = (n + 255) / 256;
  return (unsigned)(nb < 1 ? 1 : (nb < (long long)cap ? nb : (long long)cap));
}

void vs_stft_fill_shape(const vs_loss_dims* d, int B, int T, int S, VsStftShape* s);
int vs_stft_make_shape(const vs_loss_dims* d, VsStftShape* s);
VsStftLayout vs_stft_layout(const VsStftShape& s);
int vs_stft_check_envelope(const VsStftShape& s);
inline bool vs_stft_split(const VsStftShape& s) { return (size_t)s.B * s.T * s.ldk * 4 < (1ull << 32) - 4096; }
int vs_stft_contract(bool split, int layout_w, const float* A, int lda, const float* W, int ldw, float* C, int ldc, int M, int N, int K,
                     const float* a_scale2, const float* w_scale2, hipStream_t);
void vs_istft_basis_launch(float* basis, const VsStftShape& s, float* scale2, hipStream_t);
void vs_istft_envelope_launch(float* env, const VsStftShape& s, hipStream_t);
void vs_stft_basis_launch(float* basis, const VsStftShape& s, float* scale2, hipStream_t);
void vs_stft_frames_launch(const float* wav, float* frames, const VsStftShape& s, unsigned* amax, unsigned grid, hipStream_t);
void vs_spec_to_reim_launch(const float* a, const float* b, const float* phase, float* reim, const VsStftShape& s, unsigned* amax, unsigned grid,
                            hipStream_t);
void vs_overlap_add_launch(const float* frames, const float* env, float* wav, const VsStftShape& s, hipStream_t);
```

### voicesplit_amd/csrc/vs_internal.h

```cpp
#pragma once
#include "vs_common.h"

struct VsProfScope {
  hipStream_t s; int idx;
  VsProfScope(int slot, hipStream_t s);
  ~VsProfScope();
};

extern int g_vs_options[VS_OPT_COUNT];
inline int vs_opt(int o) { return g_vs_options[o]; }
extern thread_local unsigned* g_vs_turn;
struct VsTurnScope {
  unsigned* prev;
  explicit VsTurnScope(unsigned* t) : prev(g_vs_turn) { g_vs_turn = t; }
  ~VsTurnScope() { g_vs_turn = prev; }
};
inline int vs_det_grid(int nb, int cus = 256) { return (g_vs_turn && nb > cus) ? cus : nb; }

constexpr float kBnEps = 1e-5f;
constexpr float kBnMomentum = 0.1f;
struct Spec { int kt, kf, dil; };
constexpr Spec kMid[6] = {{7, 1, 1}, {5, 5, 1}, {5, 5, 2}, {5, 5, 4}, {5, 5, 8}, {5, 5, 16}};
inline size_t align_up(size_t x) { return (x + 255) & ~size_t(255); }
template <typename T>
inline T* at(void* base, size_t off) { return reinterpret_cast<T*>(static_cast<char*>(base) + off); }
template <typename T>
inline const T* at(const void* base, size_t off) { return reinterpret_cast<const T*>(static_cast<const char*>(base) + off); }
int vs_check_dims_impl(const vs_dims* d);

int vs_conv64_pack_impl(const float* w, float* wp, int KT, int KF, int transpose_flip, hipStream_t);
int vs_conv64_fwd_impl(const float* in, const float* wp, const float* scale, const float* shift, float* out,
                       int B, int T, int F, int KT, int KF, int dil, int act, hipStream_t);
int vs_pow2_scale_impl(const float* x, long long n, unsigned* amax_scratch, float* scale2, hipStream_t);
int vs_scale_from_absmax_impl(const unsigned* amax, int n, float* scale2, hipStream_t);
int vs_absmax_accum_impl(const float* x, long long n, unsigned* amax, hipStream_t);
size_t vs_gemm_presplit_bytes(int M, int N, int K);
int vs_split_rows_impl(const float* x, int rows, int K, int ld, const float* scale2, _Float16* hi, _Float16* lo, int relu, hipStream_t,
                       int math = VS_MATH_CODE_F16X3);
int vs_gemm_presplit_impl(const _Float16* Ah, const _Float16* Al, const _Float16* Wh, const _Float16* Wl, int Kp,
                          float* C, int ldc, int M, int N, const float* bias1, const float* bias2,
                          const float* rowbias, int ldrb, int group, int act, int accumulate,
                          const float* a_scale2, const float* w_scale2, hipStream_t, int math = VS_MATH_CODE_F16X3);
int vs_gemm_f16x3_impl(int layout_a, int layout_w, const float* A, int lda, const float* W, const float* W_hi,
                       int n_split, int ldw, float* C, int ldc, int M, int N, int K,
                       const float* bias1, const float* bias2, const float* rowbias, int ldrb, int group,
                       const float* gate, int ldg, int a_relu, int w_relu, int act, int accumulate,
                       const float* a_scale2, const float* w_scale2, hipStream_t, int math = VS_MATH_CODE_F16X3);
struct VsLstmSplitLayout { int Kp; size_t na, nw, Ah, Al, Wh, Wl; };
inline VsLstmSplitLayout vs_lstm_split_layout(long long M, int K, int H) {
  const int Kp = (K + VS_GEMM_KPAD - 1) / VS_GEMM_KPAD * VS_GEMM_KPAD;
  const size_t na = align_up((size_t)M * Kp * 2), nw = align_up((size_t)8 * H * Kp * 2);
  return {Kp, na, nw,  0,  na,  2 * na,  2 * na + nw};
}
bool vs_lstm_rows_fit(int M, int K, int H, const void* scratch, size_t scratch_bytes, bool prepared);
struct VsLstmGemmReady {
  const float* wscale2 = nullptr;
  const _Float16 *wh = nullptr, *wl = nullptr;
  bool feat_bf16 = false;
  bool feat_rows = false;
};
int vs_lstm_input_gemm_impl(int math, const float* feat, int K, const float* w_ih0, const float* w_ih1, int H, int KE,
                            float* xg, int M, const float* rowbias, int T, float* gemm_scales,
                            void* scratch, size_t scratch_bytes, hipStream_t, const VsLstmGemmReady& ready = VsLstmGemmReady());
int vs_lstm_split_wih_impl(int math, const float* w_ih0, const float* w_ih1, int H, int K, int KE, unsigned* amax1,
                           float* w_scale2, _Float16* Wh, _Float16* Wl, hipStream_t);
int vs_conv64_pack_f16_impl(const float* w, _Float16* wp, int KT, int KF, int transpose_flip, unsigned* amax_scratch,
                            float* w_scale2, hipStream_t);
int vs_conv64_f16x3_fwd_impl(const float* in, const _Float16* wp, const float* scale, const float* shift,
                             const float* in_scale2, const float* w_scale2, float* out,
                             int B, int T, int F, int KT, int KF, int dil, int act, unsigned* amax_out, hipStream_t,
                             double* bn_stats = nullptr);
int vs_conv64_f16x3_pk_impl(const float* in, const _Float16* wp, const float* scale, const float* shift,
                            const float* in_scale2, const float* w_scale2, float* out,
                            int B, int T, int F, int dil, int act, unsigned* amax_out, hipStream_t, int ablation = 0,
                            int i_end = 0x7fffffff, double* bn_stats = nullptr);
#define VS_SCALE_SLOT_FLOATS (8 + VS_AMAX_SLOTS)
int vs_conv64_layer_impl(int math, const float* in, const float* w, void* packed, float* slot, int in_amax_ready,
                         const float* scale, const float* shift, float* out, int B, int T, int F, int KT, int KF,
                         int dil, int act, int transpose_flip, unsigned* amax_out, hipStream_t,
                         double* bn_stats = nullptr);
inline unsigned* vs_amax_slot(float* slot) { return reinterpret_cast<unsigned*>(slot + 8); }
size_t vs_nhwc_packed_bytes(int KT, int KF);
int vs_nhwc_pack_impl(const float* w, void* packed, int KT, int KF, int transpose_flip, hipStream_t);
int vs_nhwc_conv_impl(const void* in, const void* packed, const float* scale, const float* shift, void* out,
                      int B, int T, int F, int KT, int KF, int dil, int act, double* bn_stats, hipStream_t);
size_t vs_nhwc_f16x3_packed_bytes(int KT, int KF);
int vs_nhwc_f16x3_pack_impl(const float* w, const float* w_scale2, void* packed, float* l1, int KT, int KF, hipStream_t);
int vs_nhwc_f16x3_plan_impl(const float* in_scale2, const float* w_scale2, const unsigned* amax_in, int n_amax, const float* bn_scale,
                            const float* bn_shift, const float* l1, float* eff_scale, float* eff_shift, float* out_scale2, hipStream_t);
int vs_nhwc_conv_f16x3_impl(const void* in_hi, const void* in_lo, const void* packed, const float* scale, const float* shift,
                            const float* out_scale2, void* out_hi, void* out_lo, unsigned* amax_out,
                            int B, int T, int F, int KT, int KF, int dil, int act, hipStream_t);
int vs_f16x3_split_impl(const float* x, const float* scale2, void* hi, void* lo, long long n, hipStream_t);
int vs_f16x3_merge_impl(const void* hi, const void* lo, const float* scale2, float* x, long long n, hipStream_t);
size_t vs_nhwc_f16x3_layer_scratch_bytes(int KT, int KF);
size_t vs_nhwc_f16x3_wpart_bytes(int KT, int KF);
int vs_nhwc_f16x3_prepare_wpart_impl(const float* w, void* wpart, int KT, int KF, hipStream_t);
int vs_nhwc_f16x3_layer_impl(const void* in_hi, const void* in_lo, const float* in_scale2, const unsigned* amax_in, int n_amax,
                             const float* w, const float* bn_scale, const float* bn_shift, void* wpart, int packed_ready, float* plan,
                             void* out_hi, void* out_lo, float* out_scale2, unsigned* amax_out,
                             int B, int T, int F, int KT, int KF, int dil, int act, hipStream_t);
int vs_absmax_any_impl(const float* x, long long n, unsigned* amax, hipStream_t);
int vs_nhwc_first_plan_impl(const unsigned* amax_in, int n_amax, const float* w, const float* scale, const float* shift, float* out_scale2, hipStream_t);
int vs_nhwc_conv_first_split_impl(const float* x, const float* w, const float* scale, const float* shift, const float* out_scale2,
                                  void* out_hi, void* out_lo, unsigned* amax_out, int B, int T, int F, int act, hipStream_t);
int vs_nhwc_last_plan_impl(const unsigned* amax_in, int n_amax, const float* w, const float* scale, const float* shift, float* out_scale2, hipStream_t);
int vs_nhwc_conv_last_split_impl(const void* in_hi, const void* in_lo, const float* in_scale2, const float* w, const float* scale,
                                 const float* shift, float* out, int B, int T, int F, int act, hipStream_t,
                                 void* row_hi = nullptr, void* row_lo = nullptr, int Kp = 0, const float* out_scale2 = nullptr);
#define VS_NHWC_WGRAD_MAX_PAIRS 128
size_t vs_nhwc_wgrad_partial_floats(int KT, int KF);
int vs_nhwc_wgrad_impl(const void* dz, const void* a_in, float* part, float* dw, int B, int T, int F, int KT, int KF, int dil, hipStream_t);
int vs_nhwc_conv_first_impl(const float* x, const float* w, const float* scale, const float* shift, void* out,
                            int B, int T, int F, int act, double* bn_stats, hipStream_t,
                            const float* bias = nullptr );
#define VS_FIRST_MOMENTS 35
#define VS_FIRST_BWD_SCRATCH_DOUBLES (64 * 9 + VS_FIRST_MOMENTS)
int vs_nhwc_first_moments_impl(const float* x, int B, int T, int F, double* mom, hipStream_t, double* det_slots = nullptr, int mom_is_zero = 0);
int vs_nhwc_first_stats_impl(const double* mom, const float* w, const float* bias, double count, double* stats, hipStream_t);
int vs_nhwc_first_bwd_impl(const void* da, const float* x, const float* w, const float* bias, int B, int T, int F, int act, int train,
                           const float* scale, const float* shift, const float* mean, const float* invstd,
                           float* dgamma, float* dbeta, float* dbias, float* dw, double* scratch, hipStream_t,
                           const double* moments = nullptr , double* det_slots = nullptr);
int vs_nhwc_bn_apply_impl(const void* z, void* a, long long npix, int act, const float* scale, const float* shift, hipStream_t);
int vs_nhwc_conv_last_impl(const void* in, const float* w, const float* scale, const float* shift, float* out,
                           int B, int T, int F, int act, hipStream_t, double* bn_stats = nullptr,
                           const float* pre_scale = nullptr, const float* pre_shift = nullptr, int pre_act = VS_ACT_NONE,
                           void* rows_bf16 = nullptr ,
                           int Kp = 0);
int vs_nhwc_bn_act_bwd_impl(const void* da, const void* z, void* dz, long long npix, int act, int train,
                            const float* scale, const float* shift, const float* mean, const float* invstd,
                            float* dgamma, float* dbeta, float* dbias, double* stats, float* coef, hipStream_t, int beside_wgrad = 0);
int vs_nhwc_bn_act_bwd_first_impl(const void* da, const void* z, const float* x, int B, int T, int F, int act, int train,
                                  const float* scale, const float* shift, const float* mean, const float* invstd,
                                  float* dgamma, float* dbeta, float* dbias, float* dw, double* stats, float* coef, double* acc, hipStream_t);
#define VS_NHWC_LAST_BWD_BLOCKS 1024
int vs_nhwc_conv_last_bwd_impl(const float* dz8, const float* w, const void* a7, void* din, float* part, float* dw,
                               int B, int T, int F, const void* z7, int act, const float* bn_scale, const float* bn_shift,
                               const float* bn_mean, const float* bn_invstd, double* bn_stats, hipStream_t stream);
int vs_nhwc_conv_dy_impl(const void* dz, const void* packed, void* dy, const void* z, int act,
                         const float* bn_scale, const float* bn_shift, const float* bn_mean, const float* bn_invstd, double* bn_stats,
                         int B, int T, int F, int KT, int KF, int dil, hipStream_t stream);
int vs_nhwc_bn_bwd_from_dy_impl(const void* dy, const void* z, void* dz, long long npix, int train,
                                const float* scale, const float* mean, const float* invstd,
                                float* dgamma, float* dbeta, float* dbias, double* stats, float* coef, hipStream_t stream, int rezero_doubles = 0,
                                int beside_wgrad = 0 );
int vs_nhwc_bn_bwd_first_from_dy_impl(const void* dy, const void* z, const float* x, int B, int T, int F, int train,
                                      const float* scale, const float* mean, const float* invstd,
                                      float* dgamma, float* dbeta, float* dbias, float* dw, double* stats, float* coef, double* acc,
                                      hipStream_t stream);
int vs_bn_bwd_finalize_impl(double* stats, int slots, double count, int train, int C, const float* scale, const float* mean,
                            const float* invstd, float* dgamma, float* dbeta, float* dbias, float* coef, hipStream_t,
                            int rezero_doubles = 0 );
int vs_bn_finalize_impl(double* stats, int slots, double count, int C, const float* gamma, const float* beta,
                        float* running_mean, float* running_var, float eps, float momentum,
                        float* scale, float* shift, float* mean_out, float* invstd_out, hipStream_t, int rezero_doubles = 0);
int vs_bn_fold_impl(const float*, const float*, const float*, const float*, const float*, float, int, float*, float*, hipStream_t);
int vs_conv_first_fwd_impl(const float*, const float*, const float*, const float*, float*, int, int, int, int, unsigned* amax_out, hipStream_t);
int vs_conv_last_fwd_impl(const float*, const float*, const float*, const float*, float*, int, int, int, int, hipStream_t);
int vs_bn_train_impl(const float* x, float* y, int B, int C, int plane, const float* gamma, const float* beta,
                     float* running_mean, float* running_var, float eps, float momentum, int act, double* stats,
                     float* scale, float* shift, float* mean_out, float* invstd_out, unsigned* amax_out, hipStream_t,
                     int stats_slots = 0);
int vs_bn_train_feat_impl(const float* x, float* y, int B, int T, int F, const float* gamma, const float* beta,
                          float* running_mean, float* running_var, float eps, float momentum, int act, double* stats,
                          float* scale, float* shift, float* mean_out, float* invstd_out, hipStream_t);
int vs_bn_apply_impl(const float* x, float* y, int B, int C, int plane, int act, const float* scale, const float* shift, unsigned* amax_out, hipStream_t);
int vs_bn_apply_feat_impl(const float* x, float* y, int B, int T, int F, int act, const float* scale, const float* shift, hipStream_t);
int vs_bn_apply_feat_bf16_impl(const float* x, float* y, void* yb, int Kp, int B, int T, int F, int act, const float* scale, const float* shift,
                               hipStream_t);
int vs_bn_eval_consts_impl(const float* gamma, const float* beta, const float* rmean, const float* rvar, float eps, int C,
                           float* scale, float* shift, float* mean_out, float* invstd_out, hipStream_t);
int vs_conv64_wgrad_f16x3_impl(const float* dz, const float* in, const float* dz_scale2, const float* in_scale2,
                               float* part, float* dw, int B, int T, int F, int KT, int KF, int dil, hipStream_t);
int vs_conv64_wgrad_impl(const float* dz, const float* in, float* part, float* dw, int B, int T, int F, int KT, int KF, int dil, hipStream_t);
int vs_conv64_wgrad_reduce_impl(const float* part, int G, int NT, float* dw, const float* dz_scale2 , const float* in_scale2, hipStream_t);
int vs_bn_act_bwd_impl(const float* da, const float* z, float* dz, int C, long long R, int L, int act, int train,
                       const float* scale, const float* shift, const float* mean, const float* invstd,
                       float* dgamma, float* dbeta, float* dbias, double* stats, float* coef, unsigned* amax_out, hipStream_t);
int vs_bn_act_bwd_first_impl(const float* da, const float* z, const float* x, float* xpad, int B, int T, int F, int act, int train,
                             const float* scale, const float* shift, const float* mean, const float* invstd,
                             float* dgamma, float* dbeta, float* dbias, float* dw, double* stats, float* coef, double* acc,
                             hipStream_t stream);
int vs_conv_last_dgrad_impl(const float* dz, const float* w, float* din, int B, int T, int F, hipStream_t);
int vs_conv_last_wgrad_impl(const float* dz, const float* in, float* part, float* dw, int B, int T, int F, hipStream_t);
int vs_conv_first_wgrad_impl(const float* dz, const float* x, double* acc, float* dw, int B, int T, int F, hipStream_t);
int vs_reduce_partials_impl(const float* part, int G, int n, float* out, hipStream_t);
int vs_gemm_general_impl(int layout_a, int layout_w, const float* A, int lda, const float* W, const float* W_hi,
                         int n_split, int ldw, float* C, int ldc, int M, int N, int K,
                         const float* bias1, const float* bias2, const float* rowbias, int ldrb, int group,
                         const float* gate, int ldg, int a_relu, int w_relu, int act, int accumulate,
                         int w_shift, int w_group, int splits, float* partials, hipStream_t);
int vs_gemm_general_bf16_impl(int layout_a, int layout_w, const float* A, int lda, const float* W, const float* W_hi,
                         int n_split, int ldw, float* C, int ldc, int M, int N, int K,
                         const float* bias1, const float* bias2, const float* rowbias, int ldrb, int group,
                         const float* gate, int ldg, int a_relu, int w_relu, int act, int accumulate,
                         int w_shift, int w_group, int splits, float* partials, hipStream_t);
int vs_gemm_nt_impl(const float*, int, const float*, int, float*, int, int, int, int, const float*, const float*, const float*, int, int, int, int, hipStream_t);
bool vs_head_fused_supported(int K1, int FC1, int FC2);
size_t vs_head_fused_packed_bytes(int K1, int FC1, int FC2);
int vs_head_fused_pack_impl(const float* w1, const float* b1, const float* w2, const float* b2, int K1, int FC1, int FC2, void* packed, hipStream_t);
int vs_head_fused_impl(const float* lstm_out, const void* packed, float* h1_out, float* logits, float* mask,
                       int M, int K1, int FC1, int FC2, hipStream_t);
int vs_gemm_nt_bf16_impl(const float*, int, const float*, int, float*, int, int, int, int, const float*, const float*, const float*, int, int, int, int, hipStream_t);
int vs_gemm_nt2_impl(const float*, int, const float*, const float*, int, int, float*, int, int, int, int, const float*, const float*, const float*, int, int, int, int, hipStream_t);
int vs_cvt_rows_bf16_impl(const float* src, long long rows, int K, int ld, void* dst, int Kp, hipStream_t);
int vs_gemm_bf16_impl(int a_kmajor, int b_kmajor, const void* A, int lda, const void* B, int ldb, float* C, int ldc, float* C2, int split_m,
                      int M, int N, int K, const float* rowbias, int ldrb, int group, int accumulate, hipStream_t,
                      const float* gate = nullptr, int ldg = 0);
struct VsLstmBf16Layout { size_t feat, wih, dxg, total; int Kp; };
inline VsLstmBf16Layout vs_lstm_bf16_layout(long long M, int K, int H) {
  VsLstmBf16Layout L;
  L.Kp = (K + 63) / 64 * 64;
  L.feat = 0;
  L.wih = align_up((size_t)M * L.Kp * 2);
  L.dxg = L.wih + align_up((size_t)8 * H * L.Kp * 2);
  L.total = L.dxg + align_up((size_t)M * 8 * H * 2);
  return L;
}
int vs_lstm_pack_impl(const float*, const float*, float*, int, hipStream_t, int math = VS_MATH_CODE_FP32);
struct VsLstmCarry {
  const float* state_in;
  float* state_out;
  int keep;
};
int vs_bilstm_recurrent_impl(const float* xg, const float* wp, float* state, float* out, float* gates_save, float* c_save,
                             int B, int T, int H, hipStream_t, int math = VS_MATH_CODE_FP32,
                             const int* lengths = nullptr ,
                             const float* rowbias = nullptr ,
                             int K = 1,
                             const VsLstmCarry* carry = nullptr );
int vs_lstm_carry_check(int math, int H, int T, int keep, const float* state_out, const char* what);
int vs_lstm_kernel_mode();
int vs_lstm_poison_impl(const unsigned* err, float* out, long long n, hipStream_t);
int vs_lstm_pack_t_impl(const float*, const float*, float*, int, hipStream_t, int math = VS_MATH_CODE_FP32);
int vs_bilstm_bwd_recurrent_impl(const float* wpt, float* state, float* gates, const float* c_all, const float* dout,
                                 int B, int T, int H, hipStream_t, int math = VS_MATH_CODE_FP32);
int vs_sigmoid_bwd_impl(const float* dmask, const float* mask, float* dlogits, long long n, hipStream_t);
int vs_sigmoid_bwd_rows_impl(const float* dmask, const float* mask, float* dlogits, long long rows, int N, void* rows_bf16, int Kp, hipStream_t);
int vs_cvt_f64_f32_impl(const double* src, float* dst, int n, hipStream_t);
int vs_colsum_impl(const float* x, int ld, int groups, int rows, int N, float* out, int ldo, hipStream_t);
int vs_zero_tail_rows_impl(void* ptr, int B, int T, size_t row_bytes, const int* lengths, hipStream_t, int share = 1);
```

### voicesplit_amd/losses.py

```python
import ctypes

import torch

from . import _lib
from .ops import _dev_check, _p, _stream

_WS = {}


def loss_dims(B, T, F, audio_cfg) -> "_lib.VsLossDims":
    return _lib.VsLossDims(int(B), int(T), int(F), int(audio_cfg["n_fft"]), int(audio_cfg["hop_length"]),
                           int(audio_cfg["win_length"]), float(audio_cfg.get("min_level_db", -100.0)),
                           float(audio_cfg.get("ref_level_db", 20.0)))


def _workspace(d, device):
    lib = _lib.load()
    n = lib.vs_sisnr_workspace_bytes(ctypes.byref(d))
    if n == 0:
        _lib.check(-1, "vs_sisnr_workspace_bytes")
    key = torch.device(device).index
    ws = _WS.get(key)
    if ws is None or ws.numel() < n:
        _WS.pop(key, None)
        ws = torch.empty(n, dtype=torch.uint8, device=device)
        _WS[key] = ws
    return ws


class _SiSnr(torch.autograd.Function):
    @staticmethod
    def forward(ctx, mask, mixed, target, phase, seq_len, d, want_wav):
        lib = _lib.load()
        for n, t in (("mask", mask), ("mixed", mixed), ("target", target), ("phase", phase)):
            _dev_check(t.detach(), n)
        if seq_len is not None:
            seq_len = seq_len.to(device=mask.device, dtype=torch.int32).contiguous()
        ws = _workspace(d, mask.device)
        loss = torch.empty((), dtype=torch.float32, device=mask.device)
        dmask = torch.empty_like(mask) if ctx.needs_input_grad[0] else None
        wav = torch.empty(d.B, d.hop * (d.T - 1), device=mask.device) if want_wav else None
        with torch.cuda.device(mask.device):
            rc = lib.vs_sisnr_loss(ctypes.byref(d), _p(mixed), _p(mask.detach()), _p(target), _p(phase), _p(seq_len), _p(ws),
                                   ws.numel(), _p(loss), _p(dmask), _p(wav), _stream())
        _lib.check(rc, "vs_sisnr_loss")
        ctx.dmask = dmask
        ctx.mark_non_differentiable(wav) if wav is not None else None
        return (loss, wav) if want_wav else loss

    @staticmethod
    def backward(ctx, grad_loss, *unused):
        return ctx.dmask * grad_loss, None, None, None, None, None, None


def sisnr_loss(mask, mixed, target, phase, seq_len, audio_cfg, return_wav: bool = False):
    B, T, F = mask.shape
    d = loss_dims(B, T, F, audio_cfg)
    return _SiSnr.apply(mask.contiguous(), mixed.contiguous(), target.contiguous(), phase.contiguous(), seq_len, d, return_wav)


class _PowerLaw(torch.autograd.Function):
    @staticmethod
    def forward(ctx, mask, mixed, target, power, ratio):
        lib = _lib.load()
        for n, t in (("mask", mask), ("mixed", mixed), ("target", target)):
            _dev_check(t.detach(), n)
        if mixed.shape != mask.shape or target.shape != mask.shape:
            raise ValueError(f"power_law_loss: shapes differ: mask {tuple(mask.shape)}, mixed {tuple(mixed.shape)}, "
                             f"target {tuple(target.shape)}")
        scratch = torch.empty(2, dtype=torch.float64, device=mask.device)
        loss = torch.empty((), dtype=torch.float32, device=mask.device)
        dmask = torch.empty_like(mask) if ctx.needs_input_grad[0] else None
        with torch.cuda.device(mask.device):
            rc = lib.vs_powerlaw_loss(_p(mixed), _p(mask.detach()), _p(target), mask.numel(), float(power), float(ratio),
                                      _p(scratch), _p(loss), _p(dmask), _stream())
        _lib.check(rc, "vs_powerlaw_loss")
        ctx.dmask = dmask
        return loss

    @staticmethod
    def backward(ctx, grad_loss):
        return ctx.dmask * grad_loss, None, None, None, None


def power_law_loss(mask, mixed, target, power: float = 0.3, complex_loss_ratio: float = 0.113):
    return _PowerLaw.apply(mask.contiguous(), mixed.contiguous(), target.contiguous(), power, complex_loss_ratio)
```

Measured before the change: 1449.

## Cache iSTFT tables across calls and batch both loss sides into single launches

The SI-SNR loss now builds the iSTFT basis and envelope in one kernel that checks a shape signature in the workspace and skips the rebuild when it matches. That kernel also zeroes the amax and moment buffers, replacing two memsets. The mixed and target sides are processed together: one spec-to-reim kernel, one batched scale kernel, one batched GEMM over a grid y dimension, and one overlap-add over a grid z dimension. The aim is to cut kernel launches and redundant table computation in the loss path, in exchange for reliance on a persistent workspace cache and a single-block table kernel.

```diff
diff --git a/voicesplit_amd/csrc/audio.hip b/voicesplit_amd/csrc/audio.hip
--- a/voicesplit_amd/csrc/audio.hip
+++ b/voicesplit_amd/csrc/audio.hip
@@ -41,7 +41,7 @@
   const bool split = vs_stft_split(s);
   unsigned* amax = at<unsigned>(ws, L.amax);
   float* scales = at<float>(ws, L.scales);
-  if (split) VS_CHECK_HIP(hipMemsetAsync(amax, 0, (size_t)VS_AMAX_SLOTS * 4, stream));
+  VS_CHECK_HIP(vs_stft_reset_ctl(ws, L, split ? 1 : 0, stream));
   vs_stft_frames_launch(wav, frames, s, split ? amax : nullptr, vs_grid_for((long long)M * s.win, split ? 2048 : 16384), stream);
   vs_stft_basis_launch(basis, s, scales + 6, stream);
   if (split) if (int rc = vs_scale_from_absmax_impl(amax, VS_AMAX_SLOTS, scales, stream)) return rc;
@@ -72,7 +72,7 @@
   float* scales = at<float>(ws, L.scales);
   vs_istft_basis_launch(basis, s, scales + 6, stream);
   vs_istft_envelope_launch(env, s, stream);
-  if (split) VS_CHECK_HIP(hipMemsetAsync(amax, 0, (size_t)VS_AMAX_SLOTS * 4, stream));
+  VS_CHECK_HIP(vs_stft_reset_ctl(ws, L, split ? 1 : 0, stream));
   vs_spec_to_reim_launch(spec, mask, phase, reim, s, split ? amax : nullptr, vs_grid_for((long long)M * s.F, split ? 2048 : 16384), stream);
   if (split) if (int rc = vs_scale_from_absmax_impl(amax, VS_AMAX_SLOTS, scales, stream)) return rc;
   if (int rc = vs_stft_contract(split, 0, reim, s.ldk, basis, s.ldk, frames, s.win, M, s.win, s.K, scales, scales + 6, stream)) return rc;
diff --git a/voicesplit_amd/csrc/conv_f16x3.hip b/voicesplit_amd/csrc/conv_f16x3.hip
--- a/voicesplit_amd/csrc/conv_f16x3.hip
+++ b/voicesplit_amd/csrc/conv_f16x3.hip
@@ -21,6 +21,8 @@
 }
 
 __global__ void scale_from_absmax_kernel(const unsigned* __restrict__ amax, int n, float* __restrict__ scale) {
+  amax += (size_t)blockIdx.x * n;
+  scale += 2 * blockIdx.x;
   unsigned mb = 0;
   for (int i = threadIdx.x; i < n; i += 64) mb = amax[i] > mb ? amax[i] : mb;
 #pragma unroll
@@ -339,8 +341,8 @@
 
 extern "C" size_t vs_conv64_packed_f16_floats(int KT, int KF) { return (size_t)(kNChunk * KT * KF + kPadTaps) * (kTapBytes / 4); }
 
-int vs_scale_from_absmax_impl(const unsigned* amax, int n, float* scale2, hipStream_t stream) {
-  hipLaunchKernelGGL(scale_from_absmax_kernel, dim3(1), dim3(64), 0, stream, amax, n, scale2);
+int vs_scale_from_absmax_impl(const unsigned* amax, int n, float* scale2, hipStream_t stream, int count) {
+  hipLaunchKernelGGL(scale_from_absmax_kernel, dim3(count), dim3(64), 0, stream, amax, n, scale2);
   VS_LAUNCH_CHECK();
   return 0;
 }
diff --git a/voicesplit_amd/csrc/gemm_f16x3.hip b/voicesplit_amd/csrc/gemm_f16x3.hip
--- a/voicesplit_amd/csrc/gemm_f16x3.hip
+++ b/voicesplit_amd/csrc/gemm_f16x3.hip
@@ -29,6 +29,7 @@
   const float* w_scale;
   int tiles_m, tiles_n;
   int band;
+  long long batch_a, batch_c;
 };
 
 template <bool BF = false>
@@ -157,6 +158,9 @@
   int tile_m, tile_n;
   if (!gemm_tile_of(g.tiles_m, g.tiles_n, g.band, tile_m, tile_n)) return;
   const int m0 = tile_m * BM, n0 = tile_n * BN;
+  g.A += blockIdx.y * g.batch_a;
+  g.C += blockIdx.y * g.batch_c;
+  g.a_scale += 2 * blockIdx.y;
   const float sa = g.a_scale[0], sw = g.w_scale[0];
   const float inv = g.a_scale[1] * g.w_scale[1];
 
@@ -437,8 +441,9 @@
                        int n_split, int ldw, float* C, int ldc, int M, int N, int K,
                        const float* bias1, const float* bias2, const float* rowbias, int ldrb, int group,
                        const float* gate, int ldg, int a_relu, int w_relu, int act, int accumulate,
-                       const float* a_scale2, const float* w_scale2, hipStream_t stream, int math) {
+                       const float* a_scale2, const float* w_scale2, hipStream_t stream, int math, int batch, size_t a_stride, size_t c_stride) {
   const bool bf = math == VS_MATH_CODE_BF16;
+  VS_REQUIRE(batch >= 1 && batch <= 65535, "gemm_f16x3: batch=%d", batch);
   VS_REQUIRE(M > 0 && N > 0 && K > 0, "gemm_f16x3: bad shape M=%d N=%d K=%d", M, N, K);
   VS_REQUIRE((layout_a == 0 || layout_a == 1) && (layout_w == 0 || layout_w == 1), "gemm_f16x3: bad layout");
   VS_REQUIRE(lda >= (layout_a ? M : K) && ldw >= (layout_w ? N : K) && ldc >= N,
@@ -452,12 +457,13 @@
   VS_REQUIRE(!layout_a || ((size_t)(K - 1) * lda + M) * 4 < (1ull << 32), "gemm_f16x3: K-major A above 4 GiB");
   VS_REQUIRE(!layout_w || ((size_t)(K - 1) * ldw + N) * 4 < (1ull << 32), "gemm_f16x3: K-major W above 4 GiB");
   Gemm16Args g{A, lda, W, ldw, W_hi, n_split, C, ldc, M, N, K, bias1, bias2, rowbias, ldrb, group > 0 ? group : 1,
-               gate, ldg, a_relu, w_relu, act, accumulate, a_scale2, w_scale2, (M + BM - 1) / BM, (N + BN - 1) / BN, gemm_band()};
-  const bool vec = (lda % 4 == 0) && (ldw % 4 == 0) && (K % 4 == 0) && aligned16(A) && aligned16(W) && aligned16(W_hi);
+               gate, ldg, a_relu, w_relu, act, accumulate, a_scale2, w_scale2, (M + BM - 1) / BM, (N + BN - 1) / BN, gemm_band(),
+               (long long)a_stride, (long long)c_stride};
+  const bool vec = (lda % 4 == 0) && (ldw % 4 == 0) && (K % 4 == 0) && aligned16(A) && aligned16(W) && aligned16(W_hi) && a_stride % 4 == 0;
   VS_REQUIRE(layout_a || ((size_t)(M - 1) * lda + K) * 4 < (1ull << 32) - 64, "gemm_f16x3: A above 4 GiB");
   VS_REQUIRE(layout_w || ((size_t)(N - 1) * ldw + K) * 4 < (1ull << 32) - 64, "gemm_f16x3: W above 4 GiB");
   VS_REQUIRE((long long)g.tiles_m * g.tiles_n < (1LL << 30), "gemm_f16x3: too many tiles");
-  dim3 grid((unsigned)((g.tiles_m * g.tiles_n + 7) / 8 * 8));
+  dim3 grid((unsigned)((g.tiles_m * g.tiles_n + 7) / 8 * 8), (unsigned)batch);
   if (layout_a == 0 && layout_w == 0) launch_layout<0, 0>(g, vec, grid, stream, bf);
   else if (layout_a == 0 && layout_w == 1) launch_layout<0, 1>(g, vec, grid, stream, bf);
   else if (layout_a == 1 && layout_w == 0) launch_layout<1, 0>(g, vec, grid, stream, bf);
diff --git a/voicesplit_amd/csrc/griffin_lim.hip b/voicesplit_amd/csrc/griffin_lim.hip
--- a/voicesplit_amd/csrc/griffin_lim.hip
+++ b/voicesplit_amd/csrc/griffin_lim.hip
@@ -182,7 +182,7 @@
   vs_istft_basis_launch(basis, s, scales + 4, stream);
   vs_stft_basis_launch(fbasis, s, scales + 6, stream);
   vs_istft_envelope_launch(env, s, stream);
-  if (split) VS_CHECK_HIP(hipMemsetAsync(amax, 0, (size_t)2 * VS_AMAX_SLOTS * 4, stream));
+  VS_CHECK_HIP(vs_stft_reset_ctl(ws, L, split ? 2 : 0, stream));
   VS_CHECK_HIP(hipMemsetAsync(den, 0, (size_t)s.B * 8, stream));
   VS_CHECK_HIP(hipMemsetAsync(vmax, 0, (size_t)s.B * 4, stream));
   const bool want_res = residual != nullptr && n_iter > 0;
diff --git a/voicesplit_amd/csrc/loss.hip b/voicesplit_amd/csrc/loss.hip
--- a/voicesplit_amd/csrc/loss.hip
+++ b/voicesplit_amd/csrc/loss.hip
@@ -187,24 +187,22 @@
   const bool split = vs_stft_split(s);
   unsigned* amax = at<unsigned>(ws, L.amax);
   float* scales = at<float>(ws, L.scales);
-  vs_istft_basis_launch(basis, s, scales + 6, stream);
-  vs_istft_envelope_launch(env, s, stream);
+  unsigned* ctl = at<unsigned>(ws, L.ctl);
+  double* mom = at<double>(ws, L.mom);
+  float* coef = at<float>(ws, L.coef);
+  vs_istft_tables_launch(ctl, basis, env, scales + 6, s, amax, split ? 3 * VS_AMAX_SLOTS : 0, reinterpret_cast<unsigned*>(mom), s.B * 8 * 2, stream);
   float* reim[2] = {at<float>(ws, L.reim_e), at<float>(ws, L.reim_t)};
   float* frames[2] = {at<float>(ws, L.frames_e), at<float>(ws, L.frames_t)};
   float* wav[2] = {at<float>(ws, L.wav_e), at<float>(ws, L.wav_t)};
-  if (split) VS_CHECK_HIP(hipMemsetAsync(amax, 0, (size_t)3 * VS_AMAX_SLOTS * 4, stream));
   const unsigned cap = split ? 2048 : 16384;
-  vs_spec_to_reim_launch(mixed, mask, phase, reim[0], s, split ? amax : nullptr, vs_grid_for(nspec, cap), stream);
-  vs_spec_to_reim_launch(target, nullptr, phase, reim[1], s, split ? amax + VS_AMAX_SLOTS : nullptr, vs_grid_for(nspec, cap), stream);
-  for (int q = 0; q < 2; ++q) {
-    if (split) if (int rc = vs_scale_from_absmax_impl(amax + q * VS_AMAX_SLOTS, VS_AMAX_SLOTS, scales + 2 * q, stream)) return rc;
-    if (int rc = vs_stft_contract(split, 0, reim[q], s.ldk, basis, s.ldk, frames[q], s.win, M, s.win, s.K, scales + 2 * q, scales + 6, stream)) return rc;
-    vs_overlap_add_launch(frames[q], env, wav[q], s, stream);
-  }
+  const VsReimSides sides{{mixed, target}, {mask, nullptr}, {reim[0], reim[1]},
+                          {split ? amax : nullptr, split ? amax + VS_AMAX_SLOTS : nullptr}};
+  vs_spec_to_reim_sides_launch(sides, 2, phase, s, vs_grid_for(nspec, cap), stream);
+  if (split) if (int rc = vs_scale_from_absmax_impl(amax, VS_AMAX_SLOTS, scales, stream, 2)) return rc;
+  if (int rc = vs_stft_contract(split, 0, reim[0], s.ldk, basis, s.ldk, frames[0], s.win, M, s.win, s.K, scales, scales + 6, stream,
+                                2, (size_t)(reim[1] - reim[0]), (size_t)(frames[1] - frames[0]))) return rc;
+  vs_overlap_add_launch(frames[0], env, wav[0], s, stream, 2, (size_t)(frames[1] - frames[0]), (size_t)(wav[1] - wav[0]));
   if (est_wav) VS_CHECK_HIP(hipMemcpyAsync(est_wav, wav[0], (size_t)s.B * s.S * 4, hipMemcpyDeviceToDevice, stream));
-  double* mom = at<double>(ws, L.mom);
-  float* coef = at<float>(ws, L.coef);
-  VS_CHECK_HIP(hipMemsetAsync(mom, 0, (size_t)s.B * 8 * 8, stream));
   const int gx = vs_opt(VS_OPT_DETERMINISTIC) ? 1 : (s.S + 256 * 16 - 1) / (256 * 16);
   hipLaunchKernelGGL(sisnr_moments_kernel, dim3(gx, s.B), dim3(256), 0, stream, wav[0], wav[1], seq_len, mom, s);
   hipLaunchKernelGGL(sisnr_finalize_kernel, dim3(1), dim3(64), 0, stream, mom, seq_len, coef, loss, s);
diff --git a/voicesplit_amd/csrc/stft.hip b/voicesplit_amd/csrc/stft.hip
--- a/voicesplit_amd/csrc/stft.hip
+++ b/voicesplit_amd/csrc/stft.hip
@@ -5,15 +5,13 @@
 
 namespace {
 
-__global__ void istft_basis_kernel(float* __restrict__ basis, VsStftShape s, float* __restrict__ scale2 = nullptr) {
-  const int idx = blockIdx.x * blockDim.x + threadIdx.x;
-  if (idx == 0 && scale2) {
-    int e = 0;
-    (void)frexpf(2.0f / (float)s.n_fft, &e);
-    scale2[0] = ldexpf(1.f, 10 - e);
-    scale2[1] = ldexpf(1.f, e - 10);
-  }
-  if (idx >= s.win * s.ldk) return;
+__device__ __forceinline__ void istft_basis_scale(const VsStftShape& s, float* __restrict__ scale2) {
+  int e = 0;
+  (void)frexpf(2.0f / (float)s.n_fft, &e);
+  scale2[0] = ldexpf(1.f, 10 - e);
+  scale2[1] = ldexpf(1.f, e - 10);
+}
+__device__ __forceinline__ float istft_basis_at(int idx, const VsStftShape& s) {
   const int j = idx / s.ldk, k = idx - j * s.ldk;
   float v = 0.f;
   if (k < s.K) {
@@ -25,12 +23,16 @@
     const float c = (kk == 0 || 2 * kk == s.n_fft) ? 1.0f : 2.0f;
     v = (k < s.F ? cs : -sn) * c / (float)s.n_fft * hann_w(j, s);
   }
-  basis[idx] = v;
-}
-
-__global__ void istft_envelope_kernel(float* __restrict__ env, VsStftShape s) {
-  const int sp = blockIdx.x * blockDim.x + threadIdx.x;
-  if (sp >= s.S) return;
+  return v;
+}
+__global__ void istft_basis_kernel(float* __restrict__ basis, VsStftShape s, float* __restrict__ scale2 = nullptr) {
+  const int idx = blockIdx.x * blockDim.x + threadIdx.x;
+  if (idx == 0 && scale2) istft_basis_scale(s, scale2);
+  if (idx >= s.win * s.ldk) return;
+  basis[idx] = istft_basis_at(idx, s);
+}
+
+__device__ __forceinline__ float istft_envelope_at(int sp, const VsStftShape& s) {
   const int off = s.lead;
   float e = 0.f;
   int t_hi = (sp + off) / s.hop;
@@ -41,30 +43,62 @@
     const float w = hann_w(j, s);
     e = fmaf(w, w, e);
   }
-  env[sp] = e;
+  return e;
+}
+__global__ void istft_envelope_kernel(float* __restrict__ env, VsStftShape s) {
+  const int sp = blockIdx.x * blockDim.x + threadIdx.x;
+  if (sp >= s.S) return;
+  env[sp] = istft_envelope_at(sp, s);
+}
+
+constexpr unsigned kTablesMagic = 0x69535446u;
+__global__ __launch_bounds__(1024)
+void istft_tables_kernel(unsigned* __restrict__ ctl, float* __restrict__ basis, float* __restrict__ env, float* __restrict__ scale2,
+                         VsStftShape s, unsigned* __restrict__ z0, int n0, unsigned* __restrict__ z1, int n1) {
+  const int tid = threadIdx.x;
+  const unsigned want[8] = {kTablesMagic, (unsigned)s.n_fft, (unsigned)s.hop, (unsigned)s.win, (unsigned)s.T, (unsigned)s.F,
+                            (unsigned)s.periodic, (unsigned)s.S};
+  bool hit = true;
+#pragma unroll
+  for (int i = 0; i < 8; ++i) hit = hit && ctl[i] == want[i];
+  for (int i = tid; i < n0; i += 1024) z0[i] = 0u;
+  for (int i = tid; i < n1; i += 1024) z1[i] = 0u;
+  if (hit) return;
+  for (int i = tid; i < s.win * s.ldk; i += 1024) basis[i] = istft_basis_at(i, s);
+  for (int i = tid; i < s.S; i += 1024) env[i] = istft_envelope_at(i, s);
+  if (tid == 0) istft_basis_scale(s, scale2);
+  __threadfence();
+  __syncthreads();
+  if (tid < 8) ctl[tid] = want[tid];
 }
 
 __global__ __launch_bounds__(256)
-void spec_to_reim_kernel(const float* __restrict__ a, const float* __restrict__ b, const float* __restrict__ phase,
-                         float* __restrict__ reim, VsStftShape s, unsigned* __restrict__ amax = nullptr) {
+void spec_to_reim_kernel(VsReimSides sides, int n_sides, const float* __restrict__ phase, VsStftShape s) {
   const long long n = (long long)s.B * s.T * s.F;
-  float mx = 0.f;
+  float mx[2] = {0.f, 0.f};
   for (long long i = (long long)blockIdx.x * 256 + threadIdx.x; i < n; i += (long long)gridDim.x * 256) {
     const long long m = i / s.F;
     const int f = (int)(i - m * s.F);
-    float v = a[i];
-    if (b) v *= b[i];
-    const float db = (fminf(fmaxf(v, 0.f), 1.f) - 1.f) * (-s.min_level_db) + s.ref_level_db;
-    const float mag = expf(db * kLn10Over20);
     float sn, cs;
     sincosf(phase[i], &sn, &cs);
-    const float re = s.true_phase ? mag * cs : mag * expf(cs), im = s.true_phase ? mag * sn : mag * expf(sn);
-    reim[m * s.ldk + f] = re;
-    reim[m * s.ldk + s.F + f] = im;
-    if (f == 0) for (int c = s.K; c < s.ldk; ++c) reim[m * s.ldk + c] = 0.f;
-    mx = fmaxf(mx, fmaxf(fabsf(re), fabsf(im)));
-  }
-  vs_absmax_commit(mx, amax);
+    const float pre = s.true_phase ? cs : expf(cs), pim = s.true_phase ? sn : expf(sn);
+#pragma unroll
+    for (int q = 0; q < 2; ++q) {
+      if (q >= n_sides) break;
+      float v = sides.a[q][i];
+      if (sides.b[q]) v *= sides.b[q][i];
+      const float db = (fminf(fmaxf(v, 0.f), 1.f) - 1.f) * (-s.min_level_db) + s.ref_level_db;
+      const float mag = expf(db * kLn10Over20);
+      const float re = mag * pre, im = mag * pim;
+      float* __restrict__ reim = sides.reim[q];
+      reim[m * s.ldk + f] = re;
+      reim[m * s.ldk + s.F + f] = im;
+      if (f == 0) for (int c = s.K; c < s.ldk; ++c) reim[m * s.ldk + c] = 0.f;
+      mx[q] = fmaxf(mx[q], fmaxf(fabsf(re), fabsf(im)));
+    }
+  }
+  vs_absmax_commit(mx[0], sides.amax[0]);
+  if (n_sides > 1) vs_absmax_commit(mx[1], sides.amax[1]);
 }
 
 __global__ __launch_bounds__(256)
@@ -99,10 +133,13 @@
 }
 
 __global__ __launch_bounds__(256)
-void overlap_add_kernel(const float* __restrict__ frames, const float* __restrict__ env, float* __restrict__ wav, VsStftShape s) {
+void overlap_add_kernel(const float* __restrict__ frames, const float* __restrict__ env, float* __restrict__ wav, VsStftShape s,
+                        size_t frames_stride, size_t wav_stride) {
   const int sp = blockIdx.x * 256 + threadIdx.x;
   const int b = blockIdx.y;
   if (sp >= s.S) return;
+  frames += blockIdx.z * frames_stride;
+  wav += blockIdx.z * wav_stride;
   wav[(size_t)b * s.S + sp] = stft_gather(frames, b, sp, s) / env[sp];
 }
 
@@ -120,12 +157,20 @@
 void vs_stft_frames_launch(const float* wav, float* frames, const VsStftShape& s, unsigned* amax, unsigned grid, hipStream_t stream) {
   hipLaunchKernelGGL(stft_frames_kernel, dim3(grid), dim3(256), 0, stream, wav, frames, s, amax);
 }
+void vs_spec_to_reim_sides_launch(const VsReimSides& sides, int n_sides, const float* phase, const VsStftShape& s, unsigned grid, hipStream_t stream) {
+  hipLaunchKernelGGL(spec_to_reim_kernel, dim3(grid), dim3(256), 0, stream, sides, n_sides, phase, s);
+}
 void vs_spec_to_reim_launch(const float* a, const float* b, const float* phase, float* reim, const VsStftShape& s, unsigned* amax, unsigned grid,
                             hipStream_t stream) {
-  hipLaunchKernelGGL(spec_to_reim_kernel, dim3(grid), dim3(256), 0, stream, a, b, phase, reim, s, amax);
-}
-void vs_overlap_add_launch(const float* frames, const float* env, float* wav, const VsStftShape& s, hipStream_t stream) {
-  hipLaunchKernelGGL(overlap_add_kernel, dim3((s.S + 255) / 256, s.B), dim3(256), 0, stream, frames, env, wav, s);
+  vs_spec_to_reim_sides_launch(VsReimSides{{a, a}, {b, b}, {reim, reim}, {amax, amax}}, 1, phase, s, grid, stream);
+}
+void vs_overlap_add_launch(const float* frames, const float* env, float* wav, const VsStftShape& s, hipStream_t stream, int n_sides,
+                           size_t frames_stride, size_t wav_stride) {
+  hipLaunchKernelGGL(overlap_add_kernel, dim3((s.S + 255) / 256, s.B, n_sides), dim3(256), 0, stream, frames, env, wav, s, frames_stride, wav_stride);
+}
+void vs_istft_tables_launch(unsigned* ctl, float* basis, float* env, float* scale2, const VsStftShape& s, unsigned* z0, int n0, unsigned* z1,
+                            int n1, hipStream_t stream) {
+  hipLaunchKernelGGL(istft_tables_kernel, dim3(1), dim3(1024), 0, stream, ctl, basis, env, scale2, s, z0, n0, z1, n1);
 }
 
 void vs_stft_fill_shape(const vs_loss_dims* d, int B, int T, int S, VsStftShape* s) {
@@ -153,6 +198,9 @@
   size_t off = 0;
   auto take = [&](size_t bytes) { size_t o = off; off = align_up(off + bytes); return o; };
   const size_t M = (size_t)s.B * s.T;
+  L.ctl = take(VS_STFT_CTL_BYTES);
+  L.amax = take((size_t)3 * VS_AMAX_SLOTS * 4);
+  L.scales = take(4 * 2 * 4);
   L.basis = take((size_t)s.win * s.ldk * 4);
   L.fbasis = take((size_t)s.K * s.win * 4);
   L.env = take((size_t)s.S * 4);
@@ -165,8 +213,6 @@
   L.dwav = take((size_t)s.B * s.S * 4);
   L.mom = take((size_t)s.B * 8 * 8);
   L.coef = take((size_t)s.B * 8 * 4);
-  L.amax = take((size_t)3 * VS_AMAX_SLOTS * 4);
-  L.scales = take(4 * 2 * 4);
   L.total = off;
   return L;
 }
@@ -207,11 +253,13 @@
 }
 
 int vs_stft_contract(bool split, int layout_w, const float* A, int lda, const float* W, int ldw, float* C, int ldc, int M, int N, int K,
-                     const float* a_scale2, const float* w_scale2, hipStream_t stream) {
+                     const float* a_scale2, const float* w_scale2, hipStream_t stream, int batch, size_t a_stride, size_t c_stride) {
   if (split)
     return vs_gemm_f16x3_impl(0, layout_w, A, lda, W, nullptr, 0x7fffffff, ldw, C, ldc, M, N, lda,
                               nullptr, nullptr, nullptr, 0, 1, nullptr, 0, 0, 0, VS_ACT_NONE, 0, a_scale2, w_scale2, stream,
-                              VS_MATH_CODE_F16X3);
-  return vs_gemm_general_impl(0, layout_w, A, lda, W, nullptr, 0x7fffffff, ldw, C, ldc, M, N, K,
-                              nullptr, nullptr, nullptr, 0, 1, nullptr, 0, 0, 0, VS_ACT_NONE, 0, 0, 0, 1, nullptr, stream);
-}
+                              VS_MATH_CODE_F16X3, batch, a_stride, c_stride);
+  for (int q = 0; q < batch; ++q)
+    if (int rc = vs_gemm_general_impl(0, layout_w, A + q * a_stride, lda, W, nullptr, 0x7fffffff, ldw, C + q * c_stride, ldc, M, N, K,
+                                      nullptr, nullptr, nullptr, 0, 1, nullptr, 0, 0, 0, VS_ACT_NONE, 0, 0, 0, 1, nullptr, stream)) return rc;
+  return 0;
+}
diff --git a/voicesplit_amd/csrc/stft_common.h b/voicesplit_amd/csrc/stft_common.h
--- a/voicesplit_amd/csrc/stft_common.h
+++ b/voicesplit_amd/csrc/stft_common.h
@@ -12,7 +12,12 @@
   int true_phase;
 };
 
-struct VsStftLayout { size_t basis, fbasis, env, reim_e, reim_t, frames_e, frames_t, wav_e, wav_t, dwav, mom, coef, amax, scales, total; };
+struct VsStftLayout { size_t ctl, amax, scales, basis, fbasis, env, reim_e, reim_t, frames_e, frames_t, wav_e, wav_t, dwav, mom, coef, total; };
+#define VS_STFT_CTL_BYTES 256
+
+inline hipError_t vs_stft_reset_ctl(void* ws, const VsStftLayout& L, int n_amax, hipStream_t stream) {
+  return hipMemsetAsync(static_cast<char*>(ws) + L.ctl, 0, (L.amax - L.ctl) + (size_t)n_amax * VS_AMAX_SLOTS * 4, stream);
+}
 
 __device__ __forceinline__ float hann_w(int j, const VsStftShape& s) {
   const int den = s.periodic ? s.win : s.win - 1;
@@ -42,11 +47,16 @@
 int vs_stft_check_envelope(const VsStftShape& s);
 inline bool vs_stft_split(const VsStftShape& s) { return (size_t)s.B * s.T * s.ldk * 4 < (1ull << 32) - 4096; }
 int vs_stft_contract(bool split, int layout_w, const float* A, int lda, const float* W, int ldw, float* C, int ldc, int M, int N, int K,
-                     const float* a_scale2, const float* w_scale2, hipStream_t);
+                     const float* a_scale2, const float* w_scale2, hipStream_t, int batch = 1, size_t a_stride = 0, size_t c_stride = 0);
 void vs_istft_basis_launch(float* basis, const VsStftShape& s, float* scale2, hipStream_t);
 void vs_istft_envelope_launch(float* env, const VsStftShape& s, hipStream_t);
 void vs_stft_basis_launch(float* basis, const VsStftShape& s, float* scale2, hipStream_t);
 void vs_stft_frames_launch(const float* wav, float* frames, const VsStftShape& s, unsigned* amax, unsigned grid, hipStream_t);
 void vs_spec_to_reim_launch(const float* a, const float* b, const float* phase, float* reim, const VsStftShape& s, unsigned* amax, unsigned grid,
                             hipStream_t);
-void vs_overlap_add_launch(const float* frames, const float* env, float* wav, const VsStftShape& s, hipStream_t);
+struct VsReimSides { const float* a[2]; const float* b[2]; float* reim[2]; unsigned* amax[2]; };
+void vs_spec_to_reim_sides_launch(const VsReimSides& sides, int n_sides, const float* phase, const VsStftShape& s, unsigned grid, hipStream_t);
+void vs_overlap_add_launch(const float* frames, const float* env, float* wav, const VsStftShape& s, hipStream_t, int n_sides = 1,
+                           size_t frames_stride = 0, size_t wav_stride = 0);
+void vs_istft_tables_launch(unsigned* ctl, float* basis, float* env, float* scale2, const VsStftShape& s, unsigned* z0, int n0, unsigned* z1,
+                            int n1, hipStream_t);
diff --git a/voicesplit_amd/csrc/vs_internal.h b/voicesplit_amd/csrc/vs_internal.h
--- a/voicesplit_amd/csrc/vs_internal.h
+++ b/voicesplit_amd/csrc/vs_internal.h
@@ -32,7 +32,7 @@
 int vs_conv64_fwd_impl(const float* in, const float* wp, const float* scale, const float* shift, float* out,
                        int B, int T, int F, int KT, int KF, int dil, int act, hipStream_t);
 int vs_pow2_scale_impl(const float* x, long long n, unsigned* amax_scratch, float* scale2, hipStream_t);
-int vs_scale_from_absmax_impl(const unsigned* amax, int n, float* scale2, hipStream_t);
+int vs_scale_from_absmax_impl(const unsigned* amax, int n, float* scale2, hipStream_t, int count = 1 );
 int vs_absmax_accum_impl(const float* x, long long n, unsigned* amax, hipStream_t);
 size_t vs_gemm_presplit_bytes(int M, int N, int K);
 int vs_split_rows_impl(const float* x, int rows, int K, int ld, const float* scale2, _Float16* hi, _Float16* lo, int relu, hipStream_t,
@@ -45,7 +45,8 @@
                        int n_split, int ldw, float* C, int ldc, int M, int N, int K,
                        const float* bias1, const float* bias2, const float* rowbias, int ldrb, int group,
                        const float* gate, int ldg, int a_relu, int w_relu, int act, int accumulate,
-                       const float* a_scale2, const float* w_scale2, hipStream_t, int math = VS_MATH_CODE_F16X3);
+                       const float* a_scale2, const float* w_scale2, hipStream_t, int math = VS_MATH_CODE_F16X3,
+                       int batch = 1, size_t a_stride = 0, size_t c_stride = 0 );
 struct VsLstmSplitLayout { int Kp; size_t na, nw, Ah, Al, Wh, Wl; };
 inline VsLstmSplitLayout vs_lstm_split_layout(long long M, int K, int H) {
   const int Kp = (K + VS_GEMM_KPAD - 1) / VS_GEMM_KPAD * VS_GEMM_KPAD;
diff --git a/voicesplit_amd/losses.py b/voicesplit_amd/losses.py
--- a/voicesplit_amd/losses.py
+++ b/voicesplit_amd/losses.py
@@ -23,7 +23,7 @@
     ws = _WS.get(key)
     if ws is None or ws.numel() < n:
         _WS.pop(key, None)
-        ws = torch.empty(n, dtype=torch.uint8, device=device)
+        ws = torch.zeros(n, dtype=torch.uint8, device=device)
         _WS[key] = ws
     return ws
 
```

Measured after the change: 1447. About the same (-0.1%).
